# nanoshimarobot/dynamic_direct_lidar_odometry

Hardware: AMD Instinct MI355X
Metric: GICP iters/sec + ms/scan, 131k-pt source → 500k-pt submap; pose Δ vs CPU ref (higher is better)
Workload: dtype f32 search / f64 normal equations; 1 GPU; cfg3 S2M GICP: 131,072-pt 64x2048 scan -> 500,000-pt 4-keyframe submap, LM, maxCorr 2.0 m, maxIter 32, transEps 0.01; target_points=500000, parallelism=replicas x1

## Files before the change

dynamic_direct_lidar_odometry_amd/csrc/align.hip:

```cpp
#include <hip/hip_runtime.h>

#include <algorithm>
#include <array>
#include <atomic>
#include <cfloat>
#include <cmath>
#include <cstdlib>
#include <cstring>
#include <string>
#include <thread>
#include <vector>

#include "capi_internal.hpp"
#include "cellgrid.hpp"
#include "comm.hpp"

namespace {

constexpr float kSplitExtentDefault = 5.0f;
float env_float(const char* name, float dflt) {
  const char* v = dev_getenv(name);
  if (!v || !*v) return dflt;
  char* end = nullptr;
  const float f = std::strtof(v, &end);
  return (end && end != v && f >= 0.f) ? f : dflt;
}

int env_int(const char* name, int dflt) {
  const char* v = dev_getenv(name);
  return (v && *v) ? std::atoi(v) : dflt;
}

struct SearchKnobs {
  float split_extent, probe, probe_d, tri_mv, reuse_gap, reuse_gap0, reuse_rec_eps, reuse_rec_conv;
  int xcd_scan, pf_ratio, prev_window, reuse, reuse_rec0, tie_scan, tie_ab;
};
const SearchKnobs& search_knobs() {
  static const SearchKnobs k = [] {
    SearchKnobs v;
    v.split_extent = env_float("DDLO_SPLIT_EXTENT", kSplitExtentDefault);
    v.xcd_scan = env_int("DDLO_XCD_SCAN", 1);
    v.pf_ratio = env_int("DDLO_PF_RATIO", 2);
    v.prev_window = env_int("DDLO_PREV_WINDOW", 2);
    v.tri_mv = env_float("DDLO_TRI_MV", 0.2f);
    v.probe = env_float("DDLO_PROBE", 1.0f);
    v.probe_d = env_float("DDLO_PROBE_D", 0.5f);
    v.reuse = env_int("DDLO_REUSE", 1);
    v.reuse_gap = env_float("DDLO_REUSE_GAP", 0.05f);
    v.reuse_gap0 = env_float("DDLO_REUSE_GAP0", 0.f);
    v.reuse_rec0 = env_int("DDLO_REUSE_REC0", 0);
    v.reuse_rec_eps = env_float("DDLO_REUSE_REC_EPS", 0.05f);
    v.reuse_rec_conv = env_float("DDLO_REUSE_REC_CONV", 10.f);
    v.tie_ab = env_int("DDLO_TIE_AB", 0);
    v.tie_scan = env_int("DDLO_TIE_SCAN", 4);
    return v;
  }();
  return k;
}

constexpr int kMaxFirstChunk = 8;
constexpr int kMaxFixedChunk = 64;

}

float ddlo::rt::search_cap2(const gicp_params& p) {
  const double r = p.max_correspondence_distance;
  float f = (float)(r * r);
  if (!std::isfinite(f)) f = FLT_MAX;
  return std::nextafter(f, INFINITY);
}

bool ddlo::rt::grid_active(const gicp_ctx* c) {
  if (!c->grid_mode || !c->tgt.cloud) return false;
  const auto& g = c->tgt.cloud->grid;
  return g && g->ok && g->cap2 == search_cap2(c->params);
}

void ddlo::rt::finalize_job(gicp_ctx* c) {
  AlignJob& j = *c->job_host;
  j.job_full = 0;
  AlignJob probe = j;
  std::memcpy(probe.guess_R, c->job_last.guess_R, sizeof(probe.guess_R));
  std::memcpy(probe.guess_t, c->job_last.guess_t, sizeof(probe.guess_t));
  probe.job_full = c->job_last.job_full;
  probe.ticket = c->job_last.ticket;
  if (!c->job_last_valid || std::memcmp(&probe, &c->job_last, sizeof(AlignJob)) != 0) {
    j.job_full = 1;
    c->job_last = j;
    c->job_last_valid = true;
  }
}

gicp_status ddlo::rt::fill_job(gicp_ctx* c, const float* guess16, int nblocks) {
  const SearchKnobs& kn = search_knobs();
  AlignJob& j = *c->job_host;
  std::memset(&j, 0, sizeof(j));
  j.src = c->src.cloud->dev();
  j.tgt = c->tgt.cloud->dev();
  j.src_cov = c->src.cov->cov6.as<double>();
  j.tgt_cov = c->tgt.cov->cov6.as<double>();
  j.corr = c->corr.as<int>();
  j.sqd = c->sqd.as<float>();
  j.slab = c->slab.as<double>();
  j.state = c->state_dev.as<AlignState>();
  j.ticket = (++c->ticket) & ((1ull << 47) - 1);
  j.stats = c->stats_on ? c->stats.as<unsigned int>() : nullptr;
  for (int r = 0; r < 3; ++r) {
    for (int cc = 0; cc < 3; ++cc) j.guess_R[3 * r + cc] = guess16 ? (double)guess16[4 * r + cc] : (r == cc ? 1.0 : 0.0);
    j.guess_t[r] = guess16 ? (double)guess16[4 * r + 3] : 0.0;
  }
  const double r = c->params.max_correspondence_distance;
  j.max_corr2 = r * r;
  j.cap2 = search_cap2(c->params);
  j.nblocks = nblocks;
  j.fixed_iterations = c->params.fixed_iterations;
  j.max_iterations = c->params.fixed_iterations > 0 ? c->params.fixed_iterations : c->params.max_iterations;
  j.optimizer = c->params.optimizer;
  j.lm_max_iterations = c->params.lm_max_iterations;
  j.lm_init_lambda_factor = c->params.lm_init_lambda_factor;
  j.transformation_epsilon = c->params.transformation_epsilon;
  j.rotation_epsilon = c->params.rotation_epsilon;
  j.own_axis = c->own_axis;
  j.own_lo = c->own_lo;
  j.own_hi = c->own_hi;
  j.own_mod = c->own_mod;
  j.own_rem = c->own_rem;
  j.split_extent = kn.split_extent;
  j.premom = c->comm ? 1 : 0;
  j.mom = c->mom.as<double>();
  {
    const SearchLayout sl(c->src.cloud->n);
    char* u = c->search.as<char>();
    j.qstate = reinterpret_cast<float4*>(u + sl.qstate);
    j.key = reinterpret_cast<unsigned long long*>(u + sl.key);
    j.task_ctr = reinterpret_cast<unsigned*>(u + sl.ctr);
    j.tasks = reinterpret_cast<unsigned long long*>(u + sl.tasks);
    j.task_cap_r = sl.cap_r;
    j.ref = reinterpret_cast<float4*>(u + sl.ref);
    j.ref_p = reinterpret_cast<float4*>(u + sl.ref_p);
    j.sec = reinterpret_cast<unsigned*>(u + sl.sec);
    j.key2 = reinterpret_cast<unsigned long long*>(u + sl.key2);
  }
  j.xcd_scan = kn.xcd_scan;
  j.pf_ratio = kn.pf_ratio;
  j.prev_window = kn.prev_window;
  j.tri_mv = kn.tri_mv;
  j.probe2 = kn.probe * kn.probe;
  j.probe_d = kn.probe_d;
  j.reuse = kn.reuse;
  j.reuse_gap = kn.reuse_gap;
  j.reuse_gap0 = kn.reuse_gap0;
  j.cap2_d = (double)j.cap2;
  j.tri_mv_d = (double)j.tri_mv;
  j.reuse_gap_d = (double)j.reuse_gap;
  j.reuse_gap0_d = (double)j.reuse_gap0;
  j.reuse_rec0 = kn.reuse_rec0;
  j.reuse_rec_eps = kn.reuse_rec_eps;
  j.reuse_rec_conv = kn.reuse_rec_conv;
  j.tie_detect = (c->tie_exact && (c->own_axis < 0 || c->tie_tree)) ? 1 : 0;
  j.tgt_nf = NfTreeDev{nullptr, nullptr, nullptr, 0};
  j.tgt_nf_status = nullptr;
  j.tie_scan = j.tie_detect ? kn.tie_scan : 0;
  j.tie_ab = kn.tie_ab;
  if (j.tie_detect) {
    const NfTreeData* tt = c->tie_tree ? c->tie_tree.get() : c->tgt.cloud->nf.get();
    if (tt) {
      j.tgt_nf = tt->dev();
      j.tgt_nf_status = tt->status.as<int>();
    }
  }
  j.grid_on = grid_active(c) ? 1 : 0;
  if (j.grid_on) {
    j.task_cap_r = 0;
    j.grid = c->tgt.cloud->grid->dev;
    const FbLayout fl(c->src.cloud->n);
    char* u = c->fb.as<char>();
    j.fb_count = reinterpret_cast<unsigned*>(u + fl.ctr);
    j.fb_list = reinterpret_cast<int*>(u + fl.list);
    j.fb_seg_cap = fl.seg_cap;
    j.fb_mask = reinterpret_cast<unsigned short*>(u + fl.mask);
  }
  return GICP_OK;
}

namespace {

LinGeom geometry(const gicp_ctx* c) {
  LinGeom g = linearize_geometry(c->src.cloud->n, c->tgt.cloud->upper_count());
  g.state = c->state_dev.as<AlignState>();
  g.grid = grid_active(c);
  g.grid_walk = !g.grid || c->tgt.cloud->grid->dev.has_fallback != 0;
  g.fuse_lm = !c->comm && lm_fusion_enabled(g.grid && !g.grid_walk);
  return g;
}

}

gicp_status ddlo::rt::prepare_align(gicp_ctx* c) {
  if (!c->src.cloud) return fail(GICP_ENOSOURCE, "no source cloud");
  if (!c->tgt.cloud) return fail(GICP_ENOTARGET, "no target cloud");
  if (!c->src.has_cov()) {
    gicp_status s = compute_cov(c, c->src);
    if (s) return s;
  }
  if (!c->tgt.has_cov()) {
    gicp_status s = compute_cov(c, c->tgt);
    if (s) return s;
  }
  const int ns = c->src.cloud->n;
  const size_t need_corr = sizeof(int) * ns, need_sqd = sizeof(float) * ns,
               need_slab = sizeof(double) * kSlabStride * linearize_blocks(ns),
               need_search = SearchLayout(ns).total, need_fb = grid_active(c) ? FbLayout(ns).total : 0;
  if (need_corr > c->corr.bytes || need_sqd > c->sqd.bytes || need_slab > c->slab.bytes ||
      need_search > c->search.bytes || need_fb > c->fb.bytes ||
      (c->stats_on && sizeof(unsigned int) * kStatFields * (ns + 15) > c->stats.bytes)) {
    gicp_status s = drain_tail(c);
    if (s) return s;
  }
  HIP_TRY(c->corr.ensure(sizeof(int) * ns));
  HIP_TRY(c->sqd.ensure(sizeof(float) * ns));
  HIP_TRY(c->slab.ensure(sizeof(double) * kSlabStride * linearize_blocks(ns)));
  HIP_TRY(c->mom.ensure(sizeof(double) * kSlabStride));
  HIP_TRY(c->search.ensure(need_search));
  if (need_fb) HIP_TRY(c->fb.ensure(need_fb));
  if (c->tie_exact && (c->own_axis < 0 || c->tie_tree)) {
    CloudData& tc = *c->tgt.cloud;
    if (c->comm && !c->tie_tree && !tc.nf) {
      gicp_status s = ensure_nftree(c, tc, c->stream);
      if (s) return s;
    }
    const auto& nf = c->tie_tree ? c->tie_tree : tc.nf;
    if (nf && c->nf_joined.lock() != nf) {
      HIP_TRY(nftree_join(*nf, c->stream));
      c->nf_joined = nf;
    }
  }
  if (c->stats_on) {
    HIP_TRY(c->stats.ensure(sizeof(unsigned int) * kStatFields * (ns + 15)));
    HIP_TRY(hipMemsetAsync(c->stats.p, 0, c->stats.bytes, c->stream));
  }
  return GICP_OK;
}

gicp_status ddlo::rt::ensure_tie_tree(gicp_ctx* c) {
  gicp_status s = drain_tail(c);
  if (s) return s;
  s = ensure_nftree(c, *c->tgt.cloud, c->stream);
  if (s) return s;
  HIP_TRY(nftree_join(*c->tgt.cloud->nf, c->stream));
  c->nf_joined = c->tgt.cloud->nf;
  return GICP_OK;
}

gicp_status ddlo::rt::enqueue_iteration(gicp_ctx* c, const AlignJob* jd, int nblocks, AlignState* publish) {
  (void)nblocks;
  const LinGeom g = geometry(c);
  launch_linearize(c->stream, jd, g, publish);
  if (c->comm) {
    launch_mom_reduce(c->stream, jd);
    NCCL_TRY(rccl().all_reduce(c->mom.p, c->mom.p, kSlabStride, ncclFloat64, ncclSum, c->comm, c->stream));
  }
  if (!g.fuse_lm)
    launch_lm_step(c->stream, jd, c->state_dev.as<AlignState>(), c->slab.as<double>(), g.mom_blocks,
                   c->comm ? c->mom.as<double>() : nullptr, publish);
  return GICP_OK;
}

namespace {

gicp_status enqueue_chunk(gicp_ctx* c, bool with_init, int iters, int nblocks, int slot) {
  AlignJob* jd = c->job_dev.as<AlignJob>();
  if (with_init) launch_align_init(c->stream, jd, c->job_host_dev);
  for (int i = 0; i < iters; ++i) {
    gicp_status s = enqueue_iteration(c, jd, nblocks, i == iters - 1 ? c->state_host_dev + slot : nullptr);
    if (s) return s;
  }
  return GICP_OK;
}

gicp_status capture_chunk(gicp_ctx* c, bool with_init, int iters, int nblocks, int slot, hipExecGraphPair* out) {
  ++c->captures;
  HIP_TRY(hipStreamBeginCapture(c->stream, hipStreamCaptureModeThreadLocal));
  const gicp_status s = enqueue_chunk(c, with_init, iters, nblocks, slot);
  const hipError_t e = hipStreamEndCapture(c->stream, &out->g);
  if (s) return s;
  HIP_TRY(e);
  HIP_TRY(hipGraphInstantiate(&out->ge, out->g, nullptr, nullptr, 0));
  return GICP_OK;
}

void drop_pair(hipExecGraphPair& p) {
  if (p.ge) (void)hipGraphExecDestroy(p.ge);
  if (p.g) (void)hipGraphDestroy(p.g);
  p.ge = nullptr;
  p.g = nullptr;
}

void drop_set(GraphSet& gs) {
  for (auto& p : gs.first) drop_pair(p);
  gs.first.clear();
  drop_pair(gs.rest[0]);
  drop_pair(gs.rest[1]);
  gs.key.fill(-1);
}

}

void ddlo::rt::drop_graphs(gicp_ctx* c) {
  for (auto& gs : c->gsets) drop_set(gs);
  c->gsets.clear();
}

namespace {

gicp_status graph_set(gicp_ctx* c, const std::array<long long, 7>& key, int nblocks, GraphSet** out);

bool fresh_start_enabled() {
  static const bool on = [] {
    const char* v = dev_getenv("DDLO_FRESH_START");
    return !(v && *v == '0');
  }();
  return on;
}

bool fresh_start_allowed(const gicp_ctx* c, bool prev_ok, int max_it) {
  if (!prev_ok || !fresh_start_enabled() || c->job_host->job_full != 0 || max_it <= 0) return false;
  if (c->comm || c->profiling || c->stats_on) return false;
  const LinGeom g = geometry(c);
  return linearize_is_one_kernel(g) && g.fuse_lm;
}

gicp_status run_align_graph(gicp_ctx* c, int max_it, int nblocks, bool fresh, int* final_chunk) {
  const void* jd = c->job_dev.p;
  const LinGeom g = geometry(c);
  (void)nblocks;
  const std::array<long long, 7> key{{(long long)(uintptr_t)c->slab.p | (c->comm ? 1 : 0), (long long)(uintptr_t)jd,
                                      g.seed_blocks, g.scan_blocks, g.mom_blocks, g.lds_boxes,
                                      g.grid ? (g.grid_walk ? 2L : 1L) * g.lookup_blocks : 0}};
  const bool use_graph = !c->comm || c->comm_graphs;
  const int first = c->params.fixed_iterations > 0
                        ? std::max(1, std::min(max_it, kMaxFixedChunk))
                        : std::max(1, std::min({c->predicted_iters, max_it, kMaxFirstChunk}));
  GraphSet* gs = nullptr;
  if (use_graph) {
    gicp_status s = graph_set(c, key, nblocks, &gs);
    if (s) {
      drop_graphs(c);
      (void)hipGetLastError();
      if (!c->comm) return s;
      c->comm_graphs = false;
      return run_align_graph(c, max_it, nblocks, fresh, final_chunk);
    }
  }
  if (use_graph && !fresh && !gs->first[first - 1].ge) {
    gicp_status s = capture_chunk(c, true, first, nblocks, 0, &gs->first[first - 1]);
    if (s) {
      drop_graphs(c);
      return s;
    }
  }
  auto launch_chunk = [&](int k) -> gicp_status {
    const bool is_first = k == 0;
    if (is_first && fresh) {
      const AlignJob& jh = *c->job_host;
      FreshStart fs{};
      std::memcpy(fs.R, jh.guess_R, sizeof(fs.R));
      std::memcpy(fs.t, jh.guess_t, sizeof(fs.t));
      fs.ticket = jh.ticket;
      fs.job_w = c->job_dev.as<AlignJob>();
      fs.rec0 = jh.reuse && jh.reuse_rec0;
      launch_linearize_fresh(c->stream, c->job_dev.as<AlignJob>(), g, fs, first == 1 ? c->state_host_dev : nullptr);
      HIP_TRY(hipGetLastError());
      return first > 1 ? enqueue_chunk(c, false, first - 1, nblocks, 0) : GICP_OK;
    }
    if (use_graph) {
      HIP_TRY(hipGraphLaunch(is_first ? gs->first[first - 1].ge : gs->rest[k & 1].ge, c->stream));
      return GICP_OK;
    }
    return enqueue_chunk(c, is_first, is_first ? first : 1, nblocks, k & 1);
  };
  const int nchunks = 1 + (max_it - first);
  while ((int)c->chunk_ev.size() < nchunks) {
    hipEvent_t e;
    HIP_TRY(hipEventCreateWithFlags(&e, hipEventDisableTiming));
    c->chunk_ev.push_back(e);
  }
  gicp_status s = launch_chunk(0);
  if (s) return s;
  HIP_TRY(hipEventRecord(c->chunk_ev[0], c->stream));
  int launched = 1;
  if (nchunks > 1 && c->speculate) {
    s = launch_chunk(1);
    if (s) return s;
    HIP_TRY(hipEventRecord(c->chunk_ev[1], c->stream));
    launched = 2;
  }
  int k = 0;
  static const bool spin = [] {
    const char* v = dev_getenv("DDLO_SPIN_WAIT");
    return !(v && *v == '0');
  }();
  const unsigned long long ticket = c->job_host->ticket;
  for (;;) {
    if (spin) {
      static std::atomic<int> waiters{0};
      waiters.fetch_add(1, std::memory_order_relaxed);
      const volatile unsigned long long* pw = &(c->state_host + (k & 1))->pub;
      const int expect = first + k;
      hipError_t q = hipErrorNotReady;
      for (unsigned n = 1;; ++n) {
        const unsigned long long w = *pw;
        if ((w >> 17) == ticket && (((w >> 16) & 1ull) || (int)(w & 0xffffu) >= expect)) {
          q = hipSuccess;
          break;
        }
        if ((n & 63) == 0) {
          q = hipEventQuery(c->chunk_ev[k]);
          if (q != hipErrorNotReady) {
            const unsigned long long w2 = *pw;
            if (q == hipSuccess && !((w2 >> 17) == ticket && (((w2 >> 16) & 1ull) || (int)(w2 & 0xffffu) >= expect)))
              q = hipErrorUnknown;
            break;
          }
        }
        if (waiters.load(std::memory_order_relaxed) > 1) std::this_thread::yield();
      }
      waiters.fetch_sub(1, std::memory_order_relaxed);
      if (q == hipErrorUnknown) return fail(GICP_EHIP, "align chunk completed without its state publication");
      HIP_TRY(q);
    } else {
      HIP_TRY(hipEventSynchronize(c->chunk_ev[k]));
    }
    const volatile AlignState* st = c->state_host + (k & 1);
    if (st->done || k == nchunks - 1) break;
    while (launched < nchunks && launched <= k + 2) {
      s = launch_chunk(launched);
      if (s) return s;
      HIP_TRY(hipEventRecord(c->chunk_ev[launched], c->stream));
      ++launched;
    }
    ++k;
  }
  *final_chunk = k;
  c->state_slot = k & 1;
  c->tail_ev = c->chunk_ev[launched - 1];
  c->tail_pending = launched - 1 > k || spin;
  c->speculate = k > 0;
  c->predicted_iters = std::max(1, (int)((const volatile AlignState*)(c->state_host + (k & 1)))->iter);
  return GICP_OK;
}

gicp_status graph_set(gicp_ctx* c, const std::array<long long, 7>& key, int nblocks, GraphSet** out) {
  ++c->graph_clock;
  for (auto& gs : c->gsets)
    if (gs.key == key) {
      gs.last_use = c->graph_clock;
      *out = &gs;
      return GICP_OK;
    }
  GraphSet* slot = nullptr;
  if ((int)c->gsets.size() < kGraphSets) {
    c->gsets.reserve(kGraphSets);
    c->gsets.emplace_back();
    slot = &c->gsets.back();
  } else {
    slot = &c->gsets[0];
    for (auto& gs : c->gsets)
      if (gs.last_use < slot->last_use) slot = &gs;
    gicp_status s = drain_tail(c);
    if (s) return s;
    drop_set(*slot);
  }
  slot->first.resize(kMaxFixedChunk);
  gicp_status s = capture_chunk(c, false, 1, nblocks, 0, &slot->rest[0]);
  if (!s) s = capture_chunk(c, false, 1, nblocks, 1, &slot->rest[1]);
  if (s) return s;
  slot->key = key;
  slot->last_use = c->graph_clock;
  *out = slot;
  return GICP_OK;
}

gicp_status run_align_eager_profiled(gicp_ctx* c, int max_it, int nblocks) {
  AlignJob* jd = c->job_dev.as<AlignJob>();
  const size_t need = 2 * (size_t)max_it;
  while (c->prof_ev.size() < need) {
    hipEvent_t e;
    HIP_TRY(hipEventCreate(&e));
    c->prof_ev.push_back(e);
  }
  launch_align_init(c->stream, jd, c->job_host_dev);
  for (int i = 0; i < max_it; ++i) {
    HIP_TRY(hipEventRecord(c->prof_ev[2 * i], c->stream));
    LinGeom g = geometry(c);
    g.fuse_lm = false;
    launch_linearize(c->stream, jd, g);
    HIP_TRY(hipEventRecord(c->prof_ev[2 * i + 1], c->stream));
    if (c->comm) {
      launch_mom_reduce(c->stream, jd);
      NCCL_TRY(rccl().all_reduce(c->mom.p, c->mom.p, kSlabStride, ncclFloat64, ncclSum, c->comm, c->stream));
    }
    launch_lm_step(c->stream, jd, c->state_dev.as<AlignState>(), c->slab.as<double>(), g.mom_blocks,
                   c->comm ? c->mom.as<double>() : nullptr, nullptr);
  }
  HIP_TRY(hipGetLastError());
  return GICP_OK;
}

}

namespace ddlo {
bool lm_fusion_enabled(bool lookup) {
  static const int on = [] {
    const char* v = dev_getenv("DDLO_FUSE_LM");
    return v && *v ? std::atoi(v) : -1;
  }();
  return on < 0 ? lookup : on != 0;
}
}

extern "C" {

gicp_status gicp_align(gicp_ctx* c, const float* guess16, float* out16, gicp_result* res) {
  if (!c) return fail(GICP_EINVAL, "null ctx");
  bool prev_ok = c->fresh_ok;
  c->fresh_ok = false;
  c->dbg_search = false;
  bool graph_path = false;
  begin_ties(c);
  gicp_status s = set_device(c);
  if (s) return s;
  s = maybe_build_grid(c);
  if (s) return s;
  s = prepare_align(c);
  if (s) return s;
  const int ns = c->src.cloud->n;
  const int nblocks = linearize_blocks(ns);
  hipEvent_t end_ev = c->ev1;
  int reruns = 0;
  for (;;) {
    s = fill_job(c, guess16, nblocks);
    if (s) return s;
    finalize_job(c);
    JobCommit commit(c);
    const int max_it = c->job_host->max_iterations;
    const bool fresh = fresh_start_allowed(c, prev_ok, max_it);
    prev_ok = false;
    ++(fresh ? c->fresh_aligns : c->init_aligns);
    end_ev = c->ev1;
    if (c->profiling) HIP_TRY(hipEventRecord(c->ev0, c->stream));
    if (c->profiling || max_it <= 0) {
      s = max_it > 0 ? run_align_eager_profiled(c, max_it, nblocks) : GICP_OK;
      if (s) return s;
      if (max_it <= 0) launch_align_init(c->stream, c->job_dev.as<AlignJob>(), c->job_host_dev);
      HIP_TRY(hipGetLastError());
      commit.done();
      HIP_TRY(hipEventRecord(c->ev1, c->stream));
      HIP_TRY(hipMemcpyAsync(c->state_host, c->state_dev.p, sizeof(AlignState), hipMemcpyDeviceToHost, c->stream));
      HIP_TRY(hipStreamSynchronize(c->stream));
      c->state_slot = 0;
      c->tail_pending = false;
      graph_path = false;
    } else {
      int fc = 0;
      s = run_align_graph(c, max_it, nblocks, fresh, &fc);
      if (s) return s;
      commit.done();
      graph_path = true;
      end_ev = c->chunk_ev[fc];
    }
    if (!final_state(c).tie_pending || reruns > 0) break;
    s = ensure_tie_tree(c);
    if (s) return s;
    ++reruns;
  }
  const AlignState& st = final_state(c);
  c->have_align = st.iter > 0;
  c->last_nsrc = ns;
  if (out16) {
    for (int r = 0; r < 3; ++r) {
      for (int cc = 0; cc < 3; ++cc) out16[4 * r + cc] = (float)st.R[3 * r + cc];
      out16[4 * r + 3] = (float)st.t[r];
    }
    out16[12] = out16[13] = out16[14] = 0.f;
    out16[15] = 1.f;
  }
  if (res) {
    std::memset(res, 0, sizeof(*res));
    res->converged = st.converged;
    res->nr_iterations = st.nr_iterations;
    res->iterations_run = st.iter;
    res->lm_failed = st.lm_failed;
    res->lm_trials = st.lm_trials;
    res->num_correspondences = st.num_corr;
    res->final_cost = st.final_cost;
    std::memcpy(res->final_hessian, st.final_hessian, sizeof(res->final_hessian));
    res->lm_lambda = st.lambda;
    res->ties_resolved = st.ties_resolved;
    res->tie_reruns = reruns;
    if (c->profiling) {
      float ms = 0.f;
      HIP_TRY(hipEventSynchronize(end_ev));
      HIP_TRY(hipEventElapsedTime(&ms, c->ev0, end_ev));
      res->device_ms = ms;
      double tot = 0.0;
      for (int i = 0; i < st.iter; ++i) {
        float m = 0.f;
        HIP_TRY(hipEventElapsedTime(&m, c->prof_ev[2 * i], c->prof_ev[2 * i + 1]));
        tot += m;
      }
      res->linearize_ms = tot;
    }
  }
  s = check_ties(c);
  if (s) return s;
  if (st.tie_err || st.tie_pending)
    return fail(GICP_EHIP, "nanoflann tie order: a tied correspondence could not be re-run (bits " +
                               std::to_string(st.tie_err) + (st.tie_pending ? ", no tree" : "") + ")");
  if (st.lm_failed) g_last_error = "lm not converged!!";
  c->fresh_ok = graph_path && !st.tie_pending && !st.ties_resolved && !st.tie_err;
  return GICP_OK;
}

gicp_status gicp_linearize(gicp_ctx* c, const double* pose16, double* H36, double* b6, double* cost, int32_t* ncorr) {
  if (!c || !pose16) return fail(GICP_EINVAL, "null argument");
  c->fresh_ok = false;
  c->dbg_search = false;
  begin_ties(c);
  gicp_status s = set_device(c);
  if (s) return s;
  s = maybe_build_grid(c);
  if (s) return s;
  s = prepare_align(c);
  if (s) return s;
  const int ns = c->src.cloud->n;
  const int nblocks = linearize_blocks(ns);
  for (int rerun = 0;; ++rerun) {
    float g[16];
    for (int i = 0; i < 16; ++i) g[i] = 0.f;
    s = fill_job(c, g, nblocks);
    if (s) return s;
    for (int r = 0; r < 3; ++r) {
      for (int cc = 0; cc < 3; ++cc) c->job_host->guess_R[3 * r + cc] = pose16[4 * r + cc];
      c->job_host->guess_t[r] = pose16[4 * r + 3];
    }
    c->job_host->optimizer = GICP_OPT_GAUSS_NEWTON;
    c->job_host->max_iterations = 1;
    c->job_host->fixed_iterations = 1;
    finalize_job(c);
    JobCommit commit(c);
    AlignJob* jd = c->job_dev.as<AlignJob>();
    launch_align_init(c->stream, jd, c->job_host_dev);
    s = enqueue_iteration(c, jd, nblocks, nullptr);
    if (s) return s;
    HIP_TRY(hipGetLastError());
    commit.done();
    HIP_TRY(hipMemcpyAsync(c->state_host, c->state_dev.p, sizeof(AlignState), hipMemcpyDeviceToHost, c->stream));
    HIP_TRY(hipStreamSynchronize(c->stream));
    c->state_slot = 0;
    c->tail_pending = false;
    if (!final_state(c).tie_pending || rerun > 0) break;
    s = ensure_tie_tree(c);
    if (s) return s;
  }
  const AlignState& st = final_state(c);
  if (st.tie_err || st.tie_pending)
    return fail(GICP_EHIP, "nanoflann tie order: a tied correspondence could not be re-run (bits " +
                               std::to_string(st.tie_err) + ")");
  if (H36) std::memcpy(H36, st.final_hessian, sizeof(double) * 36);
  if (cost) *cost = st.final_cost;
  if (ncorr) *ncorr = st.num_corr;
  if (b6) std::memcpy(b6, st.last_b, sizeof(double) * 6);
  c->have_align = true;
  c->last_nsrc = ns;
  return GICP_OK;
}

}

gicp_status gicp_s2s_batch(int device, const gicp_params* p, const float* const* clouds, const size_t* sizes,
                           size_t stride_bytes, int nframes, int nstreams, float* out16, gicp_result* res) {
  if (!p || !clouds || !sizes || !out16 || nframes < 1 || nstreams < 1)
    return fail(GICP_EINVAL, "invalid batch arguments");
  for (int t = 0; t < nframes; ++t)
    if (!clouds[t] || sizes[t] == 0) return fail(GICP_EINVAL, "null or empty frame");
  for (int e = 0; e < 16; ++e) out16[e] = (e % 5 == 0) ? 1.f : 0.f;
  if (res) std::memset(&res[0], 0, sizeof(gicp_result));
  const int npairs = nframes - 1;
  if (npairs == 0) return GICP_OK;
  const int nthreads = std::min(nstreams, npairs);
  std::vector<gicp_status> status(nthreads, GICP_OK);
  std::vector<std::string> errors(nthreads);
  std::vector<gicp_ctx*> ctxs(nthreads, nullptr);
  for (int w = 0; w < nthreads; ++w) {
    gicp_status s = gicp_ctx_create(device, &ctxs[w]);
    if (!s) s = gicp_set_params(ctxs[w], p);
    if (!s) {
      const char* os = dev_getenv("DDLO_NF_OWN_STREAM");
      ctxs[w]->nf_same_stream = !(os && *os == '0');
    }
    if (s) {
      const std::string why = g_last_error;
      for (auto* c : ctxs)
        if (c) (void)gicp_ctx_destroy(c);
      return fail(s, why);
    }
  }
  auto worker = [&](int w) {
    const int t0 = 1 + (int)((long)npairs * w / nthreads);
    const int t1 = 1 + (int)((long)npairs * (w + 1) / nthreads);
    gicp_ctx* c = ctxs[w];
    gicp_status s = gicp_set_target(c, clouds[t0 - 1], sizes[t0 - 1], stride_bytes);
    for (int t = t0; t < t1 && !s; ++t) {
      s = set_source_impl(c, clouds[t], sizes[t], stride_bytes, 1, true);
      if (!s) s = gicp_align(c, nullptr, out16 + 16 * (size_t)t, res ? &res[t] : nullptr);
      if (!s) s = gicp_swap_source_target(c);
    }
    if (s) {
      status[w] = s;
      errors[w] = g_last_error;
    }
  };
  std::vector<std::thread> pool;
  for (int w = 1; w < nthreads; ++w) pool.emplace_back(worker, w);
  worker(0);
  for (auto& th : pool) th.join();
  for (auto* c : ctxs) (void)gicp_ctx_destroy(c);
  for (int w = 0; w < nthreads; ++w)
    if (status[w]) return fail(status[w], "s2s batch chunk " + std::to_string(w) + ": " + errors[w]);
  return GICP_OK;
}
```

dynamic_direct_lidar_odometry_amd/csrc/capi_debug.hip:

```cpp
#include <hip/hip_runtime.h>

#include <algorithm>
#include <cstddef>
#include <cstring>
#include <limits>
#include <string>
#include <vector>

#include "capi_internal.hpp"
#include "cellgrid.hpp"

extern "C" {

gicp_status gicp_debug_search_begin(gicp_ctx* c) {
  if (!c) return fail(GICP_EINVAL, "null ctx");
  c->fresh_ok = false;
  c->dbg_search = false;
  begin_ties(c);
  gicp_status s = set_device(c);
  if (s) return s;
  s = maybe_build_grid(c);
  if (s) return s;
  s = prepare_align(c);
  if (s) return s;
  const int ns = c->src.cloud->n;
  s = fill_job(c, nullptr, linearize_blocks(ns));
  if (s) return s;
  c->job_host->optimizer = GICP_OPT_GAUSS_NEWTON;
  c->job_host->max_iterations = 1 << 30;
  c->job_host->fixed_iterations = 1 << 30;
  c->job_last_valid = false;
  finalize_job(c);
  JobCommit commit(c);
  launch_align_init(c->stream, c->job_dev.as<AlignJob>(), c->job_host_dev);
  HIP_TRY(hipGetLastError());
  HIP_TRY(hipMemcpyAsync(c->state_host, c->state_dev.p, sizeof(AlignState), hipMemcpyDeviceToHost, c->stream));
  HIP_TRY(hipStreamSynchronize(c->stream));
  c->state_slot = 0;
  c->tail_pending = false;
  c->have_align = false;
  c->last_nsrc = ns;
  std::memcpy(&c->dbg_job, c->job_host, sizeof(AlignJob));
  c->dbg_search = true;
  return GICP_OK;
}

static gicp_status debug_search_job_current(gicp_ctx* c) {
  if (!c->src.cloud || !c->tgt.cloud || !c->src.has_cov() || !c->tgt.has_cov() || c->src.cloud->n != c->last_nsrc)
    return fail(GICP_ESTATE, "the clouds or covariances changed since gicp_debug_search_begin");
  const unsigned long long ticket = c->ticket;
  gicp_status s = fill_job(c, nullptr, linearize_blocks(c->src.cloud->n));
  c->ticket = ticket;
  if (s) return s;
  AlignJob& j = *c->job_host;
  j.optimizer = c->dbg_job.optimizer;
  j.max_iterations = c->dbg_job.max_iterations;
  j.fixed_iterations = c->dbg_job.fixed_iterations;
  j.job_full = c->dbg_job.job_full;
  j.ticket = c->dbg_job.ticket;
  const bool same = std::memcmp(&j, &c->dbg_job, sizeof(AlignJob)) == 0;
  std::memcpy(&j, &c->dbg_job, sizeof(AlignJob));
  if (!same) {
    c->dbg_search = false;
    return fail(GICP_ESTATE, "the ctx changed since gicp_debug_search_begin (parameters, covariances, shard, cells or tie tree): begin again");
  }
  return GICP_OK;
}

gicp_status gicp_debug_search_step(gicp_ctx* c, const double* pose16, int rec, double* H36, double* b6, double* cost,
                                   int32_t* ncorr) {
  if (!c || !pose16) return fail(GICP_EINVAL, "null argument");
  if (!c->dbg_search || !c->src.cloud || !c->tgt.cloud || c->src.cloud->n != c->last_nsrc)
    return fail(GICP_ESTATE, "gicp_debug_search_begin first");
  gicp_status s = set_device(c);
  if (s) return s;
  s = debug_search_job_current(c);
  if (s) return s;
  begin_ties(c);
  const int ns = c->src.cloud->n;
  const int nblocks = linearize_blocks(ns);
  AlignJob* jd = c->job_dev.as<AlignJob>();
  char* const sd = c->state_dev.as<char>();
  struct {
    double Rt[12];
    int done, rec;
  } w;
  for (int r = 0; r < 3; ++r) {
    for (int cc = 0; cc < 3; ++cc) w.Rt[3 * r + cc] = pose16[4 * r + cc];
    w.Rt[9 + r] = pose16[4 * r + 3];
  }
  w.done = 0;
  w.rec = rec ? 1 : 0;
  static_assert(offsetof(AlignState, t) == offsetof(AlignState, R) + 72, "R, t: 12 consecutive doubles");
  const bool may_rerun = c->job_host->tie_detect && !c->job_host->tgt_nf.nodes;
  const SearchLayout sl(ns);
  const size_t nb_state = align256(sizeof(AlignState)), nb_corr = align256(sizeof(int) * (size_t)ns),
               nb_search = sl.tasks;
  if (may_rerun) HIP_TRY(c->dbg_snap.ensure(nb_state + 2 * nb_corr + nb_search));
  char* const snap = c->dbg_snap.as<char>();
  auto carry = [&](bool save) -> gicp_status {
    const struct {
      void* p;
      size_t off, n;
    } part[4] = {{c->state_dev.p, 0, sizeof(AlignState)},
                 {c->corr.p, nb_state, sizeof(int) * (size_t)ns},
                 {c->sqd.p, nb_state + nb_corr, sizeof(float) * (size_t)ns},
                 {c->search.p, nb_state + 2 * nb_corr, nb_search}};
    for (const auto& q : part)
      HIP_TRY(hipMemcpyAsync(save ? (void*)(snap + q.off) : q.p, save ? q.p : (void*)(snap + q.off), q.n,
                             hipMemcpyDeviceToDevice, c->stream));
    return GICP_OK;
  };
  for (int rerun = 0;; ++rerun) {
    if (may_rerun) {
      s = carry(rerun == 0);
      if (s) return s;
    }
    HIP_TRY(hipMemcpyAsync(sd + offsetof(AlignState, R), w.Rt, sizeof(w.Rt), hipMemcpyHostToDevice, c->stream));
    HIP_TRY(hipMemcpyAsync(sd + offsetof(AlignState, done), &w.done, sizeof(int), hipMemcpyHostToDevice, c->stream));
    HIP_TRY(hipMemcpyAsync(sd + offsetof(AlignState, rec), &w.rec, sizeof(int), hipMemcpyHostToDevice, c->stream));
    s = enqueue_iteration(c, jd, nblocks, nullptr);
    if (s) return s;
    HIP_TRY(hipGetLastError());
    HIP_TRY(hipMemcpyAsync(c->state_host, c->state_dev.p, sizeof(AlignState), hipMemcpyDeviceToHost, c->stream));
    HIP_TRY(hipStreamSynchronize(c->stream));
    c->state_slot = 0;
    if (!final_state(c).tie_pending || rerun > 0 || !may_rerun) break;
    s = ensure_tie_tree(c);
    if (s) return s;
    const NfTreeData* tt = c->tgt.cloud->nf.get();
    c->job_host->tgt_nf = tt->dev();
    c->job_host->tgt_nf_status = tt->status.as<int>();
    HIP_TRY(hipMemcpyAsync(reinterpret_cast<char*>(jd) + offsetof(AlignJob, tgt_nf_status), &c->job_host->tgt_nf_status,
                           sizeof(c->job_host->tgt_nf_status), hipMemcpyHostToDevice, c->stream));
    HIP_TRY(hipMemcpyAsync(reinterpret_cast<char*>(jd) + offsetof(AlignJob, tgt_nf), &c->job_host->tgt_nf,
                           sizeof(NfTreeDev), hipMemcpyHostToDevice, c->stream));
    std::memcpy(&c->dbg_job, c->job_host, sizeof(AlignJob));
  }
  const AlignState& st = final_state(c);
  s = check_ties(c);
  if (s) return s;
  if (st.tie_err || st.tie_pending)
    return fail(GICP_EHIP, "nanoflann tie order: a tied correspondence could not be re-run (bits " +
                               std::to_string(st.tie_err) + ")");
  if (H36) std::memcpy(H36, st.final_hessian, sizeof(double) * 36);
  if (cost) *cost = st.final_cost;
  if (ncorr) *ncorr = st.num_corr;
  if (b6) std::memcpy(b6, st.last_b, sizeof(double) * 6);
  c->have_align = true;
  return GICP_OK;
}

gicp_status gicp_debug_search_state(gicp_ctx* c, int32_t* corr, float* sqd, uint32_t* sec, float* ref4, float* refp4,
                                    float* wr, int32_t* any_rec_out, size_t n) {
  if (!c) return fail(GICP_EINVAL, "null ctx");
  if (!c->have_align || !c->src.cloud || !c->tgt.cloud) return fail(GICP_ESTATE, "no linearization");
  if ((int)n != c->src.cloud->n || c->last_nsrc != (int)n) return fail(GICP_EINVAL, "n != source size");
  gicp_status s = set_device(c);
  if (s) return s;
  const SearchLayout sl(c->src.cloud->n);
  if (c->search.bytes < sl.total) return fail(GICP_ESTATE, "no search state");
  const int nt = c->tgt.cloud->n;
  std::vector<int> sperm(n), tperm((size_t)nt), hcorr(n);
  std::vector<float> hsqd(n);
  std::vector<unsigned> hsec(n);
  std::vector<float4> href(n), hrefp(n), hq(n);
  const char* u = c->search.as<char>();
  HIP_TRY(hipStreamSynchronize(c->stream));
  int any_rec = 0;
  HIP_TRY(hipMemcpy(&any_rec, c->state_dev.as<char>() + offsetof(AlignState, any_rec), sizeof(int), hipMemcpyDeviceToHost));
  if (any_rec_out) *any_rec_out = any_rec;
  HIP_TRY(hipMemcpy(sperm.data(), c->src.cloud->perm.p, sizeof(int) * n, hipMemcpyDeviceToHost));
  HIP_TRY(hipMemcpy(tperm.data(), c->tgt.cloud->perm.p, sizeof(int) * (size_t)nt, hipMemcpyDeviceToHost));
  HIP_TRY(hipMemcpy(hcorr.data(), c->corr.p, sizeof(int) * n, hipMemcpyDeviceToHost));
  HIP_TRY(hipMemcpy(hsqd.data(), c->sqd.p, sizeof(float) * n, hipMemcpyDeviceToHost));
  HIP_TRY(hipMemcpy(hsec.data(), u + sl.sec, sizeof(unsigned) * n, hipMemcpyDeviceToHost));
  HIP_TRY(hipMemcpy(href.data(), u + sl.ref, sizeof(float4) * n, hipMemcpyDeviceToHost));
  HIP_TRY(hipMemcpy(hrefp.data(), u + sl.ref_p, sizeof(float4) * n, hipMemcpyDeviceToHost));
  HIP_TRY(hipMemcpy(hq.data(), u + sl.qstate, sizeof(float4) * n, hipMemcpyDeviceToHost));
  for (size_t i = 0; i < n; ++i) {
    const size_t o = (size_t)sperm[i];
    if (o >= n) return fail(GICP_EHIP, "source permutation out of range");
    if (corr) corr[o] = (hcorr[i] >= 0 && hcorr[i] < nt) ? tperm[(size_t)hcorr[i]] : -1;
    if (sqd) sqd[o] = hsqd[i];
    if (sec) sec[o] = hsec[i];
    if (ref4) std::memcpy(ref4 + 4 * o, &href[i], sizeof(float4));
    if (refp4) {
      int j;
      std::memcpy(&j, &hrefp[i].w, sizeof(int));
      const int jo = (j >= 0 && j < nt) ? tperm[(size_t)j] : -1;
      refp4[4 * o] = hrefp[i].x;
      refp4[4 * o + 1] = hrefp[i].y;
      refp4[4 * o + 2] = hrefp[i].z;
      std::memcpy(refp4 + 4 * o + 3, &jo, sizeof(int));
    }
    if (wr) wr[o] = hq[i].w;
  }
  return GICP_OK;
}

gicp_status gicp_get_start_counts(gicp_ctx* c, int64_t* fresh_starts, int64_t* init_starts) {
  if (!c) return fail(GICP_EINVAL, "null ctx");
  if (fresh_starts) *fresh_starts = c->fresh_aligns;
  if (init_starts) *init_starts = c->init_aligns;
  return GICP_OK;
}

gicp_status gicp_get_lookup_stats(gicp_ctx* c, int64_t* walk_groups) {
  if (!c || !walk_groups) return fail(GICP_EINVAL, "null argument");
  *walk_groups = -1;
  if (!c->fb.p || !c->src.cloud) return GICP_OK;
  gicp_status s = set_device(c);
  if (s) return s;
  unsigned v = 0;
  const FbLayout fl(c->src.cloud->n);
  HIP_TRY(hipMemcpyAsync(&v, c->fb.as<char>() + fl.ctr + sizeof(unsigned) * kFbSegs * 32, sizeof(unsigned),
                         hipMemcpyDeviceToHost, c->stream));
  HIP_TRY(hipStreamSynchronize(c->stream));
  *walk_groups = v;
  return GICP_OK;
}

gicp_status gicp_debug_nftree(gicp_ctx* c, int side, int32_t* vind, int32_t* nodes4, float* div2, size_t cap,
                              size_t* nnodes) {
  if (!c || (side != 0 && side != 1) || !nnodes) return fail(GICP_EINVAL, "invalid argument");
  Side& sd = side == GICP_SIDE_SOURCE ? c->src : c->tgt;
  if (!sd.cloud) return fail(GICP_ESTATE, "no cloud on this side");
  gicp_status s = set_device(c);
  if (s) return s;
  s = ensure_nftree(c, *sd.cloud, c->stream);
  if (s) return s;
  const NfTreeData& t = *sd.cloud->nf;
  HIP_TRY(nftree_join(t, c->stream));
  int st[2] = {0, 0};
  HIP_TRY(hipMemcpyAsync(st, t.status.p, sizeof(st), hipMemcpyDeviceToHost, c->stream));
  HIP_TRY(hipStreamSynchronize(c->stream));
  if (st[0]) return fail(GICP_EHIP, "nanoflann tree build failed (error bits " + std::to_string(st[0]) + ")");
  *nnodes = (size_t)st[1];
  if (!vind && !nodes4 && !div2) return GICP_OK;
  if (cap < (size_t)st[1]) return fail(GICP_EINVAL, "node capacity too small");
  const int n = t.n;
  DevBuf dv, dn, df;
  HIP_TRY(dv.ensure(sizeof(int) * (size_t)n));
  HIP_TRY(dn.ensure(sizeof(int) * 4 * (size_t)st[1]));
  HIP_TRY(df.ensure(sizeof(float) * 2 * (size_t)st[1]));
  launch_nf_export(c->stream, t.dev(), t.status.as<int>(), st[1], dv.as<int>(), dn.as<int>(), df.as<float>());
  HIP_TRY(hipGetLastError());
  if (vind) HIP_TRY(hipMemcpyAsync(vind, dv.p, sizeof(int) * (size_t)n, hipMemcpyDeviceToHost, c->stream));
  if (nodes4) HIP_TRY(hipMemcpyAsync(nodes4, dn.p, sizeof(int) * 4 * (size_t)st[1], hipMemcpyDeviceToHost, c->stream));
  if (div2) HIP_TRY(hipMemcpyAsync(div2, df.p, sizeof(float) * 2 * (size_t)st[1], hipMemcpyDeviceToHost, c->stream));
  HIP_TRY(hipStreamSynchronize(c->stream));
  return GICP_OK;
}

gicp_status gicp_debug_nfbuild(gicp_ctx* c, int side, int stop, int32_t* vind, int64_t* info16, int32_t* status2,
                               void* scratch, size_t scratch_cap) {
  if (!c || (side != 0 && side != 1) || !vind || !info16 || !status2) return fail(GICP_EINVAL, "invalid argument");
  Side& sd = side == GICP_SIDE_SOURCE ? c->src : c->tgt;
  if (!sd.cloud) return fail(GICP_ESTATE, "no cloud on this side");
  gicp_status s = set_device(c);
  if (s) return s;
  NfTreeData t;
  long long off[16];
  s = nftree_build(c, *sd.cloud, c->stream, t, stop, off);
  if (s) return s;
  HIP_TRY(nftree_join(t, c->stream));
  for (int i = 0; i < 16; ++i) info16[i] = off[i];
  HIP_TRY(hipMemcpyAsync(status2, t.status.p, 2 * sizeof(int), hipMemcpyDeviceToHost, c->stream));
  std::vector<float4> v((size_t)t.n);
  HIP_TRY(hipMemcpyAsync(v.data(), t.vpts.p, sizeof(float4) * (size_t)t.n, hipMemcpyDeviceToHost, c->stream));
  if (scratch && scratch_cap)
    HIP_TRY(hipMemcpyAsync(scratch, c->nf_scratch.p, std::min(scratch_cap, (size_t)off[13]), hipMemcpyDeviceToHost,
                           c->stream));
  HIP_TRY(hipStreamSynchronize(c->stream));
  for (int i = 0; i < t.n; ++i) {
    int w;
    std::memcpy(&w, &v[(size_t)i].w, sizeof(int));
    vind[i] = w;
  }
  return GICP_OK;
}

gicp_status gicp_get_moments(const gicp_ctx* c, double* out80) {
  if (!c || !out80) return fail(GICP_EINVAL, "null argument");
  std::memcpy(out80, final_state(c).last_mom, sizeof(double) * kSlabStride);
  return GICP_OK;
}

gicp_status gicp_debug_lm_step(gicp_ctx* c, const gicp_lm_state* in, const double* slab, int nrows, const double* mom80,
                               gicp_lm_state* out) {
  if (!c || !in || !out || !slab == !mom80) return fail(GICP_EINVAL, "null argument (pass either slab or mom80)");
  const int max_rows = lm_slab_rows_max();
  if (slab && (nrows < 1 || nrows > max_rows)) return fail(GICP_EINVAL, "nrows must be in [1, 256]");
  gicp_status s = set_device(c);
  if (s) return s;
  AlignJob j{};
  j.fixed_iterations = c->params.fixed_iterations;
  j.max_iterations = c->params.fixed_iterations > 0 ? c->params.fixed_iterations : c->params.max_iterations;
  j.optimizer = c->params.optimizer;
  j.lm_max_iterations = c->params.lm_max_iterations;
  j.lm_init_lambda_factor = c->params.lm_init_lambda_factor;
  j.transformation_epsilon = c->params.transformation_epsilon;
  j.rotation_epsilon = c->params.rotation_epsilon;
  j.reuse = 0;
  AlignState st{};
  std::memcpy(st.R, in->R, sizeof(st.R));
  std::memcpy(st.t, in->t, sizeof(st.t));
  st.lambda = in->lambda;
  st.final_cost = in->final_cost;
  std::memcpy(st.final_hessian, in->final_hessian, sizeof(st.final_hessian));
  std::memcpy(st.last_b, in->last_b, sizeof(st.last_b));
  std::memcpy(st.last_mom, in->last_mom, sizeof(st.last_mom));
  st.iter = in->iter;
  st.lm_trials = in->lm_trials;
  st.converged = in->converged;
  st.lm_failed = in->lm_failed;
  st.done = 0;
  st.nr_iterations = in->nr_iterations;
  st.num_corr = in->num_corr;
  std::vector<double> rows;
  if (slab) {
    rows.assign((size_t)max_rows * kSlabStride, std::numeric_limits<double>::quiet_NaN());
    std::memcpy(rows.data(), slab, sizeof(double) * (size_t)nrows * kSlabStride);
  } else {
    rows.assign(mom80, mom80 + kSlabStride);
  }
  DevBuf djob, dstate, dmom;
  HIP_TRY(djob.ensure(sizeof(AlignJob)));
  HIP_TRY(dstate.ensure(sizeof(AlignState)));
  HIP_TRY(dmom.ensure(sizeof(double) * rows.size()));
  HIP_TRY(hipMemcpyAsync(djob.p, &j, sizeof(j), hipMemcpyHostToDevice, c->stream));
  HIP_TRY(hipMemcpyAsync(dstate.p, &st, sizeof(st), hipMemcpyHostToDevice, c->stream));
  HIP_TRY(hipMemcpyAsync(dmom.p, rows.data(), sizeof(double) * rows.size(), hipMemcpyHostToDevice, c->stream));
  launch_lm_step(c->stream, djob.as<AlignJob>(), dstate.as<AlignState>(), slab ? dmom.as<double>() : nullptr,
                 slab ? nrows : 0, slab ? nullptr : dmom.as<double>(), nullptr);
  HIP_TRY(hipGetLastError());
  HIP_TRY(hipMemcpyAsync(&st, dstate.p, sizeof(st), hipMemcpyDeviceToHost, c->stream));
  HIP_TRY(hipStreamSynchronize(c->stream));
  std::memcpy(out->R, st.R, sizeof(st.R));
  std::memcpy(out->t, st.t, sizeof(st.t));
  out->lambda = st.lambda;
  out->final_cost = st.final_cost;
  std::memcpy(out->final_hessian, st.final_hessian, sizeof(st.final_hessian));
  std::memcpy(out->last_b, st.last_b, sizeof(st.last_b));
  std::memcpy(out->last_mom, st.last_mom, sizeof(st.last_mom));
  out->iter = st.iter;
  out->lm_trials = st.lm_trials;
  out->converged = st.converged;
  out->lm_failed = st.lm_failed;
  out->done = st.done;
  out->nr_iterations = st.nr_iterations;
  out->num_corr = st.num_corr;
  out->reserved = 0;
  return GICP_OK;
}

gicp_status gicp_debug_stats(gicp_ctx* c, int enable, unsigned int* out, size_t max_words, size_t* nwords) {
  if (!c) return fail(GICP_EINVAL, "null ctx");
  c->stats_on = enable != 0;
  if (out && c->src.cloud && c->stats.p) {
    const int q = search_queries_per_wave();
    const size_t groups = (c->src.cloud->n + q - 1) / q;
    const size_t words = std::min(max_words, (size_t)kStatFields * (groups + (groups + 3) / 4));
    HIP_TRY(hipMemcpyAsync(out, c->stats.p, sizeof(unsigned int) * words, hipMemcpyDeviceToHost, c->stream));
    HIP_TRY(hipStreamSynchronize(c->stream));
    if (nwords) *nwords = words;
  }
  return GICP_OK;
}

gicp_status gicp_set_profiling(gicp_ctx* c, int enable) {
  if (!c) return fail(GICP_EINVAL, "null ctx");
  c->profiling = enable != 0;
  return GICP_OK;
}

gicp_status gicp_get_stage_times(gicp_ctx* c, gicp_stage_times* out) {
  if (!c || !out) return fail(GICP_EINVAL, "null argument");
  std::memset(out, 0, sizeof(*out));
  if (!c->st_ev[0]) return fail(GICP_ESTATE, "no profiled compute_covariances on this ctx");
  gicp_status s = set_device(c);
  if (s) return s;
  HIP_TRY(hipStreamSynchronize(c->stream));
  HIP_TRY(hipStreamSynchronize(c->aux_stream));
  float ms = 0.f;
  HIP_TRY(hipEventElapsedTime(&ms, c->st_ev[0], c->st_ev[1]));
  out->cov_ms = ms;
  if (c->st_tree) {
    HIP_TRY(hipEventElapsedTime(&ms, c->st_ev[2], c->st_ev[3]));
    out->tree_ms = ms;
  }
  if (c->st_resolve) {
    HIP_TRY(hipEventElapsedTime(&ms, c->st_ev[4], c->st_ev[5]));
    out->resolve_ms = ms;
  }
  return GICP_OK;
}

}
```

dynamic_direct_lidar_odometry_amd/csrc/capi_internal.hpp:

```cpp
#pragma once
#include "runtime.hpp"

namespace ddlo {
namespace rt {

struct SearchLayout {
  size_t qstate, key, ctr, ref, ref_p, sec, key2, tasks, total;
  int cap_r;
  explicit SearchLayout(int ns) {
    cap_r = task_cap_per_region(ns);
    qstate = 0;
    key = align256(sizeof(float4) * (size_t)ns);
    ctr = key + align256(sizeof(unsigned long long) * (size_t)ns);
    ref = ctr + align256(sizeof(unsigned) * (kTaskRegions + 1) * kCtrStride);
    ref_p = ref + align256(sizeof(float4) * (size_t)ns);
    sec = ref_p + align256(sizeof(float4) * (size_t)ns);
    key2 = sec + align256(sizeof(unsigned) * (size_t)ns);
    tasks = key2 + align256(sizeof(unsigned long long) * (size_t)ns);
    total = tasks + sizeof(unsigned long long) * (size_t)kTaskRegions * cap_r;
  }
};

struct FbLayout {
  size_t ctr, list, mask, total;
  int seg_cap;
  explicit FbLayout(int ns) {
    seg_cap = (ns + 15) / 16 + 1;
    ctr = 0;
    list = align256(sizeof(unsigned) * (kFbSegs + 1) * 32);
    mask = list + align256(sizeof(int) * (size_t)kFbSegs * seg_cap);
    total = mask + align256(sizeof(unsigned short) * (size_t)seg_cap);
  }
};


float search_cap2(const gicp_params& p);
bool grid_active(const gicp_ctx* c);

inline int linearize_blocks(int nsrc) { return linearize_geometry(nsrc, 0).mom_blocks; }

struct JobCommit {
  gicp_ctx* c;
  bool ok = false;
  explicit JobCommit(gicp_ctx* ctx) : c(ctx) {}
  void done() { ok = true; }
  ~JobCommit() {
    if (!ok) c->job_last_valid = c->fresh_ok = false;
  }
};
void finalize_job(gicp_ctx* c);
gicp_status fill_job(gicp_ctx* c, const float* guess16, int nblocks);
gicp_status prepare_align(gicp_ctx* c);
gicp_status ensure_tie_tree(gicp_ctx* c);
gicp_status enqueue_iteration(gicp_ctx* c, const AlignJob* jd, int nblocks, AlignState* publish);
void drop_graphs(gicp_ctx* c);


gicp_status set_source_impl(gicp_ctx* c, const float* xyz, size_t n, size_t stride, int build_index, bool nf_early);

}
}
```

dynamic_direct_lidar_odometry_amd/csrc/gicp_types.hpp:

```cpp
#pragma once
#include <stdint.h>

namespace ddlo {

constexpr int kLeafSize = 32;
constexpr int kFanout = 64;
constexpr int kMaxLevels = 5;
constexpr int kDirBits = 18;
constexpr int kFineBits = 6;
constexpr int kFineMin = 32;
__host__ __device__ constexpr long fine_dir_ints(int n) {
  return (1L << kDirBits) + 2 + (1L << kDirBits) + ((long)(n / (kFineMin + 1) + 1) << kFineBits) / 2;
}

constexpr int kMoments = 74;
constexpr int kMomentSlots = 96;
constexpr int kSlabStride = 80;
constexpr int kStatFields = 8;

constexpr int kTaskRegions = 64;
constexpr int kCtrStride = 32;
constexpr int kTasksPerGroup = 48;

struct CloudDev {
  const float4* pts;
  const unsigned long long* keys;
  const int* perm;
  const int* inv_perm;
  const float4* box_lo;
  const float4* box_hi;
  const float* quant;
  const float* soa;
  const int* dir;
  int n;
  int nlevels;
  int off0, off1, off2, off3, off4;
  int cnt0, cnt1, cnt2, cnt3, cnt4;
};

__host__ __device__ inline int lvl_off(const CloudDev& c, int l) {
  return l == 0 ? c.off0 : l == 1 ? c.off1 : l == 2 ? c.off2 : l == 3 ? c.off3 : c.off4;
}
__host__ __device__ inline int lvl_cnt(const CloudDev& c, int l) {
  return l == 0 ? c.cnt0 : l == 1 ? c.cnt1 : l == 2 ? c.cnt2 : l == 3 ? c.cnt3 : c.cnt4;
}

struct NfNode {
  int c1, c2;
  int feat;
  float divlow, divhigh;
  int parent;
  int pad0, pad1;
};

struct NfTreeDev {
  const float4* vpts;
  const NfNode* nodes;
  const float4* box;
  int n;
  int partial;
  const float4* sbox;
};

constexpr unsigned long long kCgNoMatch = ~0ull;
constexpr unsigned long long kCgFallback = ~0ull - 1;
constexpr unsigned kCgFineFallback = 0xffffffffu;
constexpr int kCgMaxLevel = 3;
constexpr int kCgEntPad = 32;

struct CellGridDev {
  const unsigned long long* dir;
  const uint2* fine;
  const float4* ent;
  float ox, oy, oz, inv_s;
  int nx, ny, nz;
  int outside_nomatch;
  int has_fallback;
};

__device__ __forceinline__ int cg_cell_list(const CellGridDev& G, float tx, float ty, float tz, unsigned& off,
                                            unsigned& cnt) {
  const int cx = min((int)tx, G.nx - 1), cy = min((int)ty, G.ny - 1), cz = min((int)tz, G.nz - 1);
  const unsigned long long d = G.dir[((long)cx * G.ny + cy) * G.nz + cz];
  if (d == kCgNoMatch) return 0;
  if (d == kCgFallback) return 2;
  const int lvl = (int)(d >> 62);
  unsigned long long e = d;
  if (lvl != 0) {
    const int m = 1 << lvl;
    const int fx = min((int)((tx - (float)cx) * (float)m), m - 1);
    const int fy = min((int)((ty - (float)cy) * (float)m), m - 1);
    const int fz = min((int)((tz - (float)cz) * (float)m), m - 1);
    e = reinterpret_cast<const unsigned long long*>(G.fine)[(unsigned)d + (unsigned)((fx * m + fy) * m + fz)];
  }
  if ((unsigned)(e >> 32) == kCgFineFallback) return 2;
  off = (unsigned)e;
  cnt = (unsigned)(e >> 32) & 0x3fffffffu;
  return 1;
}

struct AlignState {
  double R[9];
  double t[3];
  double lambda;
  double final_hessian[36];
  double final_cost;
  double last_lin_R[9];
  double last_lin_t[3];
  double last_b[6];
  double last_mom[kSlabStride];
  int iter;
  int done;
  int converged;
  int nr_iterations;
  int lm_failed;
  int lm_trials;
  int num_corr;
  int have_prev;
  int rec;
  float src_radius;
  int any_rec;
  int tie_pending;
  int ties_resolved;
  int tie_err;
  unsigned long long pub;
};

struct AlignJob {
  CloudDev src;
  CloudDev tgt;
  const double* src_cov;
  const double* tgt_cov;
  int* corr;
  float* sqd;
  double* slab;
  AlignState* state;
  unsigned int* stats;
  double guess_R[9];
  double guess_t[3];
  long long job_full;
  unsigned long long ticket;
  double max_corr2;
  float cap2;
  double cap2_d, tri_mv_d, reuse_gap_d, reuse_gap0_d;
  int nblocks;
  int max_iterations;
  int fixed_iterations;
  int optimizer;
  int lm_max_iterations;
  double lm_init_lambda_factor;
  double transformation_epsilon;
  double rotation_epsilon;
  int own_axis;
  float own_lo, own_hi;
  int own_mod, own_rem;
  int premom;
  double* mom;
  float split_extent;
  float4* qstate;
  unsigned long long* key;
  unsigned long long* tasks;
  unsigned* task_ctr;
  int task_cap_r;
  int xcd_scan;
  int pf_ratio;
  int prev_window;
  float probe2;
  float probe_d;
  float tri_mv;
  int reuse;
  float reuse_gap;
  float reuse_gap0;
  int reuse_rec0;
  float reuse_rec_eps;
  float reuse_rec_conv;
  float4* ref;
  float4* ref_p;
  unsigned* sec;
  unsigned long long* key2;
  int tie_detect;
  int tie_ab;
  int tie_scan;
  const int* tgt_nf_status;
  NfTreeDev tgt_nf;
  int grid_on;
  CellGridDev grid;
  unsigned* fb_count;
  int* fb_list;
  int fb_seg_cap;
  unsigned short* fb_mask;
};
constexpr int kFbSegs = 8;

struct FreshStart {
  double R[9];
  double t[3];
  unsigned long long ticket;
  AlignJob* job_w;
  int rec0;
};

constexpr int kNfMaxLevels = 40;
constexpr int kNfLevelSpare = 2;

struct NfCtl {
  int nnodes, nsmall, err;
  int nchunks[2];
  int ntask[kNfMaxLevels + 1];
  int dbg[16];
};

struct NfTask {
  int node, begin, count, chunk0;
  float lo[3], hi[3];
  unsigned mm[6];
  int feat;
  float cut;
  int nch, pad;
};

struct NfBuild {
  float4* vpts;
  NfNode* nodes;
  float4* box;
  int cap;
  NfCtl* ctl;
  NfTask* tasks;
  NfTask* pend;
  NfTask* small;
  int* chunk_task;
  NfTask* ctask;
  int *cA, *cAE, *cE2;
  float4 *tblL, *tblR;
  const float* quant;
  float4* sbox;
  const float4* sorted;
  const int* gate;
  int n, Lmax, max_task, max_pend, max_small, max_chunks;
  int nbucket;
  int big_ids;
};

struct NfSizes {
  int Lmax, max_task, max_pend, max_small, max_chunks, big_ids;
};

struct KnnJob {
  CloudDev c;
  int k;
  int method;
  double* cov6;
  float4* qstate;
  unsigned long long* cand;
  unsigned* cnt;
  int cap;
  unsigned long long* tasks;
  unsigned* task_ctr;
  int task_cap_r;
  unsigned char* redo;
  unsigned char* again;
  int round;
  int* slot2;
  unsigned long long* cand2;
  unsigned* n2;
  int cap2, max2;
  float split_extent;
  int* tie_list;
  int* tie_count;
  int tie_cap;
};

}
```

dynamic_direct_lidar_odometry_amd/csrc/launch.hpp:

```cpp
#pragma once
#include <hip/hip_runtime.h>

#include "gicp_types.hpp"

namespace ddlo {

void launch_pack_bbox(hipStream_t s, const unsigned char* raw, size_t stride, int n, float4* out, float* partial,
                      int* nonfinite, int nblocks);
void launch_bbox_final(hipStream_t s, const float* partial, int nparts, float* quant);
void launch_morton(hipStream_t s, const float4* pts, int n, const float* quant, unsigned long long* keys, int* vals);
void launch_gather(hipStream_t s, const float4* raw, const int* perm, int n, int npad, float4* sorted, int* inv_perm);
void launch_key_dir(hipStream_t s, const unsigned long long* keys, int n, int* dir);
void launch_leaf_soa_boxes(hipStream_t s, const float4* pts, int n, int nleaves, float* soa, float4* lo, float4* hi);
void launch_level_boxes(hipStream_t s, const float4* clo, const float4* chi, int nchild, int nparent, float4* plo,
                        float4* phi);
struct TieList {
  int* list;
  int* count;
  int cap = 0;
  __device__ __forceinline__ void push(int i) const {
    const int slot = atomicAdd(count, 1);
    if (slot < cap) list[slot] = i;
  }
};
bool launch_covariances(hipStream_t s, const CloudDev& c, int k, int method, double* cov6, const unsigned char* redo,
                        TieList ties = TieList{nullptr, nullptr});
bool launch_knn_covariances(hipStream_t s, const KnnJob& j, int tgt_upper);
int knn_task_cap_per_region(int n);
bool launch_knn_query(hipStream_t s, const CloudDev& c, const float4* q, int nq, int k, int* out_idx, float* out_d,
                      TieList ties = TieList{nullptr, nullptr});
void launch_cov_import(hipStream_t s, const double* in, int layout, int n, const int* inv_perm, double* cov6);
void launch_cov_export(hipStream_t s, const double* cov6, int layout, int n, const int* perm, double* out);
size_t tie_prune_scratch_bytes(int n, int cap);
hipError_t launch_tie_prune(hipStream_t s, const NfTreeDev& t, int cap, const int* local_index, int n_local,
                            void* scratch, NfNode* out_nodes, float4* out_pts, unsigned* counts);
void launch_align_init(hipStream_t s, AlignJob* job, const AlignJob* job_src);
struct LinGeom {
  int seed_blocks, scan_blocks, mom_blocks, lds_boxes, lookup_blocks;
  bool fuse_lm = false;
  AlignState* state = nullptr;
  bool grid = false;
  bool grid_walk = true;
};
bool lm_fusion_enabled(bool lookup);
LinGeom linearize_geometry(int nsrc, int tgt_upper);
void launch_linearize(hipStream_t s, const AlignJob* job, const LinGeom& g, AlignState* publish = nullptr);
bool linearize_is_one_kernel(const LinGeom& g);
void launch_linearize_fresh(hipStream_t s, const AlignJob* job, const LinGeom& g, const FreshStart& fs,
                            AlignState* publish = nullptr);
int search_queries_per_wave();
int task_cap_per_region(int nsrc);
int moment_blocks(int nsrc);
int lm_slab_rows_max();
void launch_lm_step(hipStream_t s, const AlignJob* job, AlignState* st, const double* slab, int nblocks,
                    const double* premom, AlignState* publish);
void launch_mom_reduce(hipStream_t s, const AlignJob* job);
void launch_residuals(hipStream_t s, const AlignJob* job, int nsrc, double* out);
void launch_residual_image(hipStream_t s, const float4* pts, const int* perm, const int* inv_perm, int n,
                           const double* residual, double tmin, double tmax, int W, int H, int* winner, float* img,
                           float* xyz);
void launch_transform(hipStream_t s, const float4* pts, int n, const int* perm, const float* T16, float* out,
                      size_t stride_floats);
void launch_export_corr(hipStream_t s, const AlignJob* job, int nsrc, int* corr, float* sqd);

NfSizes nf_sizes(int n);
void launch_nf_build(hipStream_t s, const NfBuild& hb, const NfBuild* db, int stop = -1);
void launch_nf_set_desc(hipStream_t s, const NfBuild& b, NfBuild* db);
void launch_nf_export(hipStream_t s, const NfTreeDev& t, const int* status, int cap, int* vind, int* nodes, float* f);
bool launch_nf_resolve_cov(hipStream_t s, const NfTreeDev& t, const CloudDev& c, TieList ties, int k, int method,
                           double* cov6, const int* status, int* err);
bool launch_nf_resolve_knn(hipStream_t s, const NfTreeDev& t, const float4* q, TieList ties, int k, int* out_idx,
                           float* out_d, const int* status, int* err);
size_t nf_lazy_bytes(int n, int wgs);
bool launch_nf_lazy(hipStream_t s, const NfTreeDev& t, const CloudDev& c, const float4* q, TieList ties, int k,
                    int method, double* cov6, int* out_idx, float* out_d, void* scratch, int wgs, const int* status,
                    int* err);
void launch_cov_remap(hipStream_t s, const double* old_cov6, const int* old_inv_perm, const int* new_perm, int n,
                      double* cov6);

void launch_pack4(hipStream_t s, const unsigned char* raw, size_t stride, int n, float4* out);
long long rowcol_size(int rows, int cols, int row_step, int col_step);
int rowcol_count(int n, int rows, int cols, int row_step, int col_step);
int launch_pack4_rowcol(hipStream_t s, const unsigned char* raw, size_t stride, int n, int rows, int cols, int row_step,
                        int col_step, float4* out);
struct CropCentre {
  float x = 0.f, y = 0.f, z = 0.f;
};
int crop_box(hipStream_t s, const float4* in, int n, float size, float4* out, int* keep, int* pos, void* tmp,
             size_t tmp_bytes, int* count_host, int* pin, CropCentre centre = CropCentre(), bool box = true);
size_t crop_box_tmp_bytes(int n);
int compact_flagged(hipStream_t s, const float4* in, int n, float4* out, const int* keep, int* pos, void* tmp,
                    size_t tmp_bytes, int* count_host, int* pin);
int voxel_grid(hipStream_t s, const float4* in, int n, float leaf, float4* out, int* scratch, void* tmp, size_t tmp_bytes,
               int* count_host, float crop, int* pin, CropCentre centre = CropCentre(), int order = 0,
               int* oscratch = nullptr);
size_t voxel_tmp_bytes(int n);
constexpr size_t voxel_scratch_ints(int n) { return 7 * (size_t)n + 16 + 6 * 64; }

constexpr int kVoxelOrderHandOver = 512;
size_t sort_order_scratch_ints(int n);
size_t voxel_order_scratch_ints(int n);
void launch_sort_order(hipStream_t s, unsigned* keys, int* idx, int n, const int* pos, const int* keep, int* scratch);
int voxel_order_pairs(hipStream_t s, const unsigned* keys, const int* idx, int n, int* oscratch, void* tmp,
                      size_t tmp_bytes, unsigned** ck_out, int** ci_out);
void median_range_async(hipStream_t s, const float4* in, int n, float* d, float* result, void* tmp, size_t tmp_bytes,
                        float* out);
size_t median_tmp_bytes(int n);
void launch_transform4(hipStream_t s, const float4* pts, const int* perm, int n, const float* T12, float4* out);
void launch_transform_raw(hipStream_t s, const unsigned char* raw, size_t stride, int n, const float* T12, float4* out);
void launch_gather_cov6(hipStream_t s, const double* cov_sorted, const int* perm, int n, double* out);

}
```

dynamic_direct_lidar_odometry_amd/csrc/lm_step.hpp:

```cpp
#pragma once
#include <hip/hip_runtime.h>

#include "gicp_types.hpp"
#include "search.hpp"

namespace ddlo {

static __device__ void so3_exp_d(const double w[3], double R[9]) {
  const double theta_sq = w[0] * w[0] + w[1] * w[1] + w[2] * w[2];
  double imag, real;
  if (theta_sq < 1e-10) {
    const double theta_quad = theta_sq * theta_sq;
    imag = 0.5 - 1.0 / 48.0 * theta_sq + 1.0 / 3840.0 * theta_quad;
    real = 1.0 - 1.0 / 8.0 * theta_sq + 1.0 / 384.0 * theta_quad;
  } else {
    const double theta = sqrt(theta_sq);
    const double half = 0.5 * theta;
    double sh, ch;
    sincos(half, &sh, &ch);
    imag = sh / theta;
    real = ch;
  }
  const double qw = real, qx = imag * w[0], qy = imag * w[1], qz = imag * w[2];
  const double tx = 2 * qx, ty = 2 * qy, tz = 2 * qz;
  const double twx = tx * qw, twy = ty * qw, twz = tz * qw;
  const double txx = tx * qx, txy = ty * qx, txz = tz * qx;
  const double tyy = ty * qy, tyz = tz * qy, tzz = tz * qz;
  R[0] = 1 - (tyy + tzz); R[1] = txy - twz;       R[2] = txz + twy;
  R[3] = txy + twz;       R[4] = 1 - (txx + tzz); R[5] = tyz - twx;
  R[6] = txz - twy;       R[7] = tyz + twx;       R[8] = 1 - (txx + tyy);
}

static __device__ void ldlt_solve6_perm(const double* H, const double* b, double lambda, double* xs, double x[6]) {
  constexpr int n = 6;
  double v[6];
  int p[6];
#pragma unroll
  for (int i = 0; i < n; ++i) {
    v[i] = fabs(H[7 * i] + lambda);
    p[i] = i;
  }
#pragma unroll
  for (int k = 0; k < n - 1; ++k) {
    double bv = v[k];
    int bp = p[k], big = k;
#pragma unroll
    for (int i = k + 1; i < n; ++i)
      if (v[i] > bv) { bv = v[i]; bp = p[i]; big = i; }
#pragma unroll
    for (int i = k + 1; i < n; ++i)
      if (big == i) { v[i] = v[k]; p[i] = p[k]; }
    v[k] = bv;
    p[k] = bp;
  }
  double m[36];
#pragma unroll
  for (int i = 0; i < n; ++i)
#pragma unroll
    for (int j = 0; j <= i; ++j) {
      const int hi = max(p[i], p[j]), lo = min(p[i], p[j]);
      m[i * n + j] = i == j ? H[7 * p[i]] + lambda : H[hi * n + lo];
    }
#pragma unroll
  for (int k = 0; k < n; ++k) {
    if (k > 0) {
      double temp[6];
#pragma unroll
      for (int j = 0; j < k; ++j) temp[j] = m[j * n + j] * m[k * n + j];
      double s = 0;
#pragma unroll
      for (int j = 0; j < k; ++j) s += m[k * n + j] * temp[j];
      m[k * n + k] -= s;
#pragma unroll
      for (int i = k + 1; i < n; ++i) {
        double a = 0;
#pragma unroll
        for (int j = 0; j < k; ++j) a += m[i * n + j] * temp[j];
        m[i * n + k] -= a;
      }
    }
    const double akk = m[k * n + k];
    if (k < n - 1 && fabs(akk) > 0.0) {
#pragma unroll
      for (int i = k + 1; i < n; ++i) m[i * n + k] /= akk;
    }
  }
  double y[6];
#pragma unroll
  for (int i = 0; i < n; ++i) y[i] = -b[p[i]];
#pragma unroll
  for (int i = 0; i < n; ++i)
#pragma unroll
    for (int j = 0; j < i; ++j) y[i] -= m[i * n + j] * y[j];
#pragma unroll
  for (int i = 0; i < n; ++i) y[i] = (fabs(m[i * n + i]) > 2.2250738585072014e-308) ? y[i] / m[i * n + i] : 0.0;
#pragma unroll
  for (int i = n - 1; i >= 0; --i)
#pragma unroll
    for (int j = i + 1; j < n; ++j) y[i] -= m[j * n + i] * y[j];
#pragma unroll
  for (int i = 0; i < n; ++i) xs[p[i]] = y[i];
#pragma unroll
  for (int i = 0; i < n; ++i) x[i] = xs[i];
}

constexpr int mom_ab(int a, int b) {
  return a <= b ? (a == 0 ? b : (a == 1 ? 2 + b : 5)) : (b == 0 ? a : (b == 1 ? 2 + a : 5));
}
constexpr int mom_w(int k, int l, int a, int b) {
  return (k == 3 && l == 3) ? mom_ab(a, b)
         : k == 3           ? 6 + 6 * l + mom_ab(a, b)
         : l == 3           ? 6 + 6 * k + mom_ab(a, b)
                            : 24 + 6 * mom_ab(k, l) + mom_ab(a, b);
}
constexpr int mom_g(int mm, int k) { return 60 + 4 * mm + k; }
constexpr int kMomY0 = 72, kMomCount = 73;

constexpr int kNeqEntries = 198;
struct NeqTerm {
  unsigned idx;
  unsigned sgn;
  unsigned ctl;
};
struct NeqTable {
  NeqTerm e[kNeqEntries];
};
constexpr void skew_nz_c(int i, int p, int& c, int& r, int& sg) {
  constexpr int cc[3][2] = {{1, 2}, {0, 2}, {0, 1}};
  constexpr int rr[3][2] = {{2, 1}, {2, 0}, {1, 0}};
  constexpr int ss[3][2] = {{-1, 1}, {1, -1}, {-1, 1}};
  c = cc[i][p];
  r = rr[i][p];
  sg = ss[i][p];
}
constexpr NeqTable make_neq_table() {
  NeqTable T{};
  auto add = [&](int e, int idx, int sg) {
    const unsigned t = T.e[e].ctl & 0xffu;
    T.e[e].idx |= (unsigned)idx << (8 * t);
    T.e[e].sgn |= (sg < 0 ? 0xffu : 1u) << (8 * t);
    T.e[e].ctl += 1u;
  };
  for (int e = 0; e < 42; ++e) {
    if (e >= 36) {
      const int i = e - 36;
      if (i >= 3) {
        add(e, mom_g(i - 3, 3), -1);
      } else {
        for (int p = 0; p < 2; ++p) {
          int c = 0, r = 0, sg = 0;
          skew_nz_c(i, p, c, r, sg);
          add(e, mom_g(r, c), sg);
        }
      }
      continue;
    }
    const int i = e / 6, j = e % 6;
    if (i < 3 && j < 3) {
      for (int p = 0; p < 2; ++p) {
        int c = 0, r = 0, sr = 0;
        skew_nz_c(i, p, c, r, sr);
        for (int u = 0; u < 2; ++u) {
          int d = 0, q = 0, sq = 0;
          skew_nz_c(j, u, d, q, sq);
          add(e, mom_w(c, d, r, q), sr * sq);
        }
      }
    } else if (i >= 3 && j >= 3) {
      add(e, mom_w(3, 3, i - 3, j - 3), 1);
    } else {
      const int a = i < 3 ? i : j, t = i < 3 ? j - 3 : i - 3;
      for (int p = 0; p < 2; ++p) {
        int c = 0, r = 0, sr = 0;
        skew_nz_c(a, p, c, r, sr);
        add(e, mom_w(c, 3, r, t), sr);
      }
      T.e[e].ctl |= 0x100u;
    }
  }
  for (int e = 0; e < 144; ++e) add(42 + e, mom_w(e / 12 / 3, e % 12 / 3, e / 12 % 3, e % 12 % 3), 1);
  for (int e = 0; e < 12; ++e) add(186 + e, mom_g(e % 3, e / 3), 1);
  return T;
}
static __constant__ NeqTable kNeq = make_neq_table();
__device__ __forceinline__ double neq_term(const NeqTerm& E, const double* mom, int t) {
  const double v = mom[(E.idx >> (8 * t)) & 0xffu];
  return ((E.sgn >> (8 * t)) & 0xffu) == 1u ? v : -v;
}
__device__ __forceinline__ double neq_value(const NeqTerm& E, const double* mom) {
  const unsigned n = E.ctl & 0xffu;
  double s = neq_term(E, mom, 0);
  if (n > 1) {
    s = 0.0 + s;
#pragma unroll
    for (int t = 1; t < 4; ++t)
      if (t < (int)n) s += neq_term(E, mom, t);
  }
  return (E.ctl & 0x100u) ? -s : s;
}

constexpr int kLmThreads = 512;
constexpr int kMaxTrials = 64;
constexpr int kMomBlocksMax = 256;
constexpr int kLmParts = 12;
constexpr int kLmRowsPerPart = (kMomBlocksMax + kLmParts - 1) / kLmParts;

__device__ __forceinline__ void reduce_slab(const double* slab_in, int nb, double (*part)[kSlabStride], double* mom) {
  const int tid = threadIdx.x;
  const auto slab = (const __attribute__((address_space(1))) d2v*)gp(slab_in);
  constexpr int kPairs = kSlabStride / 2;
  if (tid < kLmParts * kPairs) {
    const int v2 = tid % kPairs, p = tid / kPairs;
    d2v x[kLmRowsPerPart];
#pragma unroll
    for (int r = 0; r < kLmRowsPerPart; ++r) x[r] = slab[(size_t)min(p + kLmParts * r, nb - 1) * kPairs + v2];
    double s0 = 0.0, s1 = 0.0;
#pragma unroll
    for (int r = 0; r < kLmRowsPerPart; ++r) {
      const bool in = p + kLmParts * r < nb;
      s0 += in ? x[r].x : 0.0;
      s1 += in ? x[r].y : 0.0;
    }
    part[p][2 * v2] = s0;
    part[p][2 * v2 + 1] = s1;
  }
  __syncthreads();
  if (tid < kSlabStride) {
    double s = 0.0;
#pragma unroll
    for (int p = 0; p < kLmParts; ++p) s += part[p][tid];
    mom[tid] = s;
  }
}

#ifdef DDLO_LM_PROF
#define LM_PROF(i) if (threadIdx.x == 0) lm_t[i] = __builtin_amdgcn_s_memtime()
#define LM_PROF_TRIAL(i) if (threadIdx.x == 0) lm_tt[i] = __builtin_amdgcn_s_memtime()
#else
#define LM_PROF(i)
#define LM_PROF_TRIAL(i)
#endif
template <bool PREMOM, bool FRESH = false>
__device__ __forceinline__ void lm_step_body(const AlignJob* __restrict__ job, AlignState* __restrict__ st,
                                             const double* __restrict__ slab, int nblocks,
                                             const double* __restrict__ premom, const FreshStart* fs = nullptr) {
#ifdef DDLO_LM_PROF
  unsigned long long lm_t[6], lm_tt[4] = {0, 0, 0, 0};
#endif
  LM_PROF(0);
  __shared__ double part[kLmParts][kSlabStride];
  __shared__ double mom[kSlabStride];
  __shared__ double nq[kNeqEntries];
  double* const Hs = nq;
  double* const bs = nq + 36;
  double* const W12 = nq + 42;
  double* const g12 = nq + 186;
  __shared__ double tr_lambda[kMaxTrials], tr_cm[kMaxTrials], tr_fro[kMaxTrials];
  __shared__ double tr_R[kMaxTrials][9], tr_t[kMaxTrials][3];
  __shared__ double tr_d[kMaxTrials][12], tr_row[kMaxTrials][12], tr_den[kMaxTrials], tr_x[kMaxTrials][6];
  __shared__ double Rt_s[12];
  __shared__ int tr_conv[kMaxTrials];
  const int tid = threadIdx.x;
  const int it_pre = FRESH ? 0 : st->iter;
  const int trials_pre = FRESH ? 0 : st->lm_trials;
  const int rec_pre = FRESH ? fs->rec0 : st->rec;
  const float src_radius = st->src_radius;
  const double lambda_pre = FRESH ? -1.0 : st->lambda;
  double rt_v = 0.0;
  if constexpr (FRESH) {
#pragma unroll
    for (int e = 0; e < 12; ++e)
      if (tid == e) rt_v = e < 9 ? fs->R[e] : fs->t[e - 9];
  } else {
    if (tid < 12) rt_v = tid < 9 ? st->R[tid] : st->t[tid - 9];
  }
  const int optimizer = job->optimizer, lm_max_iterations = job->lm_max_iterations;
  const int fixed_iterations = job->fixed_iterations, max_iterations = job->max_iterations;
  const double lm_init_lambda_factor = job->lm_init_lambda_factor;
  const double rotation_epsilon = job->rotation_epsilon, transformation_epsilon = job->transformation_epsilon;
  const int reuse = job->reuse;
  const float reuse_rec_eps = job->reuse_rec_eps, reuse_rec_conv = job->reuse_rec_conv;
  NeqTerm E{};
  if (tid < kNeqEntries) E = kNeq.e[tid];
  if constexpr (PREMOM) {
    if (tid < kSlabStride) mom[tid] = gp(premom)[tid];
  } else {
    reduce_slab(slab, nblocks, part, mom);
  }
  if (tid < 12) Rt_s[tid] = rt_v;
  __syncthreads();
  LM_PROF(1);
  if (tid < kNeqEntries) nq[tid] = neq_value(E, mom);
  __syncthreads();
  LM_PROF(2);
  const bool lm = optimizer != 0;
  const int ntr = lm ? min(lm_max_iterations, kMaxTrials) : 1;
  if (tid < ntr) {
    const int trial = tid;
    double lambda = 0.0;
    if (lm) {
      lambda = lambda_pre;
      if (lambda < 0.0) {
        double mx = 0.0;
        for (int e = 0; e < 6; ++e) mx = fmax(mx, fabs(Hs[7 * e]));
        lambda = lm_init_lambda_factor * mx;
      }
      double nu = 2.0;
      for (int k = 0; k < trial; ++k) {
        lambda = nu * lambda;
        nu = 2 * nu;
      }
    }
    LM_PROF_TRIAL(0);
    double d[6];
    ldlt_solve6_perm(Hs, bs, lambda, tr_x[trial], d);
    LM_PROF_TRIAL(1);
    double Rd[9], td[3];
    so3_exp_d(d, Rd);
    LM_PROF_TRIAL(2);
    td[0] = d[3]; td[1] = d[4]; td[2] = d[5];
    double den = 0.0;
    for (int e = 0; e < 6; ++e) den += d[e] * (lambda * d[e] - bs[e]);
    tr_den[trial] = den;
    tr_lambda[trial] = lambda;
    double mr = 0.0, mt = 0.0;
    for (int i = 0; i < 3; ++i)
      for (int j = 0; j < 3; ++j) mr = fmax(mr, fabs(Rd[3 * i + j] - (i == j ? 1.0 : 0.0)));
    for (int i = 0; i < 3; ++i) mt = fmax(mt, fabs(td[i]));
    const double cm = fmax(1.0 / rotation_epsilon * mr, 1.0 / transformation_epsilon * mt);
    tr_cm[trial] = cm;
    tr_conv[trial] = fixed_iterations <= 0 && cm < 1;
    double fro = 0.0;
    for (int e = 0; e < 9; ++e) {
      const double dd = Rd[e] - ((e % 4 == 0) ? 1.0 : 0.0);
      fro += dd * dd;
    }
    tr_fro[trial] = fro;
    for (int e = 0; e < 9; ++e) tr_R[trial][e] = Rd[e];
    for (int e = 0; e < 3; ++e) tr_t[trial][e] = td[e];
#pragma unroll
    for (int k = 0; k < 4; ++k)
#pragma unroll
      for (int a = 0; a < 3; ++a) tr_d[trial][3 * k + a] = k < 3 ? Rd[3 * a + k] - (a == k ? 1.0 : 0.0) : td[a];
    LM_PROF_TRIAL(3);
  }
  __syncthreads();
  LM_PROF(3);
  for (int x = tid; lm && x < 12 * ntr; x += (int)blockDim.x) {
    const int tr = x / 12, i = x % 12;
    double srow = 0.0;
#pragma unroll
    for (int j = 0; j < 12; ++j) srow += W12[12 * i + j] * tr_d[tr][j];
    tr_row[tr][i] = tr_d[tr][i] * srow;
  }
  __syncthreads();
  LM_PROF(4);
  if (tid >= 64) {
    const int u = tid - 64;
    if (u < kSlabStride) st->last_mom[u] = mom[u];
    else if (u < kSlabStride + 9) st->last_lin_R[u - kSlabStride] = Rt_s[u - kSlabStride];
    else if (u < kSlabStride + 12) st->last_lin_t[u - kSlabStride - 9] = Rt_s[u - kSlabStride];
    else if (u < kSlabStride + 18) st->last_b[u - kSlabStride - 12] = bs[u - kSlabStride - 12];
    return;
  }
  const int lane = tid;
  double rho = 1.0;
  if (lm && lane < ntr) {
    double lin = 0.0, quad = 0.0;
#pragma unroll
    for (int r = 0; r < 3; ++r)
#pragma unroll
      for (int k = 0; k < 4; ++k) lin += tr_d[lane][3 * k + r] * g12[3 * k + r];
#pragma unroll
    for (int i = 0; i < 12; ++i) quad += tr_row[lane][i];
    rho = (2.0 * lin - quad) / tr_den[lane];
  }
  bool ok = true, accept = true;
  int chosen = 0;
  if (lm) {
    const unsigned long long ball = __ballot(lane < ntr && (!(rho < 0) || tr_conv[lane]));
    ok = ball != 0ull;
    chosen = ok ? (int)__builtin_ctzll(ball) : ntr - 1;
    const double rho_c = __shfl(rho, chosen);
    accept = ok && !(rho_c < 0);
    if (lane == 0) {
      st->lm_trials = trials_pre + (ok ? chosen + 1 : ntr);
      if (accept) {
        const double c = 2 * rho_c - 1;
        st->lambda = tr_lambda[chosen] * fmax(1.0 / 3.0, 1 - c * c * c);
      } else if (ok) {
        st->lambda = tr_lambda[chosen];
      } else {
        st->lambda = tr_lambda[ntr - 1] * 2.0;
      }
    }
  } else if (FRESH && lane == 0) {
    st->lm_trials = 0;
    st->lambda = -1.0;
  }
  if (lane == 0) {
    st->nr_iterations = it_pre;
    st->final_cost = mom[kMomY0];
    st->num_corr = (int)mom[kMomCount];
    if (rec_pre) st->any_rec = 1;
    else if (FRESH) st->any_rec = 0;
    st->iter = it_pre + 1;
    st->have_prev = 1;
    int done = 0;
    if constexpr (FRESH) {
      const int failed = !ok, conv = ok && tr_conv[chosen];
      st->lm_failed = failed;
      st->converged = conv;
      done = failed | conv;
      if (it_pre + 1 >= max_iterations) done = 1;
      st->done = done;
    } else {
      if (!ok) {
        st->lm_failed = 1;
        done = 1;
      } else if (tr_conv[chosen]) {
        st->converged = 1;
        done = 1;
      }
      if (it_pre + 1 >= max_iterations) done = 1;
      if (done) st->done = 1;
    }
  }
  double v = 0.0;
  if (accept) {
    const double* Rd = tr_R[chosen];
    if (lane < 9) {
      const int i = lane / 3, j = lane % 3;
      v = Rd[3 * i + 0] * Rt_s[0 + j] + Rd[3 * i + 1] * Rt_s[3 + j] + Rd[3 * i + 2] * Rt_s[6 + j];
      st->R[lane] = v;
    } else if (lane < 12) {
      const int i = lane - 9;
      v = (Rd[3 * i + 0] * Rt_s[9] + Rd[3 * i + 1] * Rt_s[10] + Rd[3 * i + 2] * Rt_s[11]) + tr_t[chosen][i];
      st->t[i] = v;
    } else if (lane >= 16 && lane < 16 + 36) {
      st->final_hessian[lane - 16] = Hs[lane - 16];
    }
  } else if (FRESH && lane < 12) {
    if (lane < 9) st->R[lane] = Rt_s[lane];
    else st->t[lane - 9] = Rt_s[lane];
  }
  int rec = reuse;
  if (accept) {
    const double tn0 = __shfl(v, 9), tn1 = __shfl(v, 10), tn2 = __shfl(v, 11);
    const double* dt = tr_t[chosen];
    const double mv = sqrt(tr_fro[chosen]) * ((double)src_radius + sqrt(tn0 * tn0 + tn1 * tn1 + tn2 * tn2)) +
                      sqrt(dt[0] * dt[0] + dt[1] * dt[1] + dt[2] * dt[2]);
    rec = rec && mv < (double)reuse_rec_eps && (fixed_iterations > 0 || tr_cm[chosen] > (double)reuse_rec_conv);
  }
  if (lane == 0) st->rec = rec;
  LM_PROF(5);
#ifdef DDLO_LM_PROF
  if (tid == 0)
    printf("lm_prof %d %llu %llu %llu %llu %llu %llu %llu %llu %llu\n", it_pre, lm_t[1] - lm_t[0], lm_t[2] - lm_t[1],
           lm_t[3] - lm_t[2], lm_t[4] - lm_t[3], lm_t[5] - lm_t[4], lm_tt[0] - lm_t[2], lm_tt[1] - lm_tt[0],
           lm_tt[2] - lm_tt[1], lm_tt[3] - lm_tt[2]);
#endif
}

}
```

dynamic_direct_lidar_odometry_amd/csrc/moments.hip:

```cpp
#include <hip/hip_runtime.h>

#include <cstddef>

#include "gicp_types.hpp"
#include "search.hpp"
#include "nftree.hpp"
#include "cov_math.hpp"
#include "launch.hpp"
#include "launch_util.hpp"
#include "linearize_internal.hpp"
#include "lm_step.hpp"

namespace ddlo {

struct Contrib {
  double M[6];
  double q[3];
  double qq[6];
  double v[3];
  double y;
  double c;
};

template <int S>
__device__ __forceinline__ double moment_val(const Contrib& C) {
  if constexpr (S < 6) {
    return C.M[S];
  } else if constexpr (S < 24) {
    return C.q[(S - 6) / 6] * C.M[(S - 6) % 6];
  } else if constexpr (S < 60) {
    return C.qq[(S - 24) / 6] * C.M[(S - 24) % 6];
  } else if constexpr (S < 72) {
    constexpr int m = (S - 60) / 4, kk = (S - 60) % 4;
    if constexpr (kk == 3)
      return C.v[m];
    else
      return C.v[m] * C.q[kk];
  } else if constexpr (S == 72) {
    return C.y;
  } else if constexpr (S == 73) {
    return C.c;
  } else {
    return 0.0;
  }
}

__device__ __forceinline__ double dpp_f64(double x, int ctrl_sel) {
  const int lo = __double2loint(x), hi = __double2hiint(x);
  int rlo, rhi;
  switch (ctrl_sel) {
    case 0:
      rlo = __builtin_amdgcn_update_dpp(0, lo, 0x140, 0xf, 0xf, false);
      rhi = __builtin_amdgcn_update_dpp(0, hi, 0x140, 0xf, 0xf, false);
      break;
    case 1:
      rlo = __builtin_amdgcn_update_dpp(0, lo, 0x141, 0xf, 0xf, false);
      rhi = __builtin_amdgcn_update_dpp(0, hi, 0x141, 0xf, 0xf, false);
      break;
    case 2:
      rlo = __builtin_amdgcn_update_dpp(0, lo, 0x4e, 0xf, 0xf, false);
      rhi = __builtin_amdgcn_update_dpp(0, hi, 0x4e, 0xf, 0xf, false);
      break;
    default:
      rlo = __builtin_amdgcn_update_dpp(0, lo, 0xb1, 0xf, 0xf, false);
      rhi = __builtin_amdgcn_update_dpp(0, hi, 0xb1, 0xf, 0xf, false);
      break;
  }
  return __hiloint2double(rhi, rlo);
}

template <int L>
__device__ __forceinline__ double xchg(double a, double b) {
  if constexpr (L == 1 || L == 2) {
    const unsigned alo = __double2loint(a), ahi = __double2hiint(a);
    const unsigned blo = __double2loint(b), bhi = __double2hiint(b);
    unsigned x0, x1, y0, y1;
    if constexpr (L == 1) {
      const auto rl = __builtin_amdgcn_permlane32_swap(alo, blo, false, false);
      const auto rh = __builtin_amdgcn_permlane32_swap(ahi, bhi, false, false);
      x0 = rl[0]; y0 = rl[1]; x1 = rh[0]; y1 = rh[1];
    } else {
      const auto rl = __builtin_amdgcn_permlane16_swap(alo, blo, false, false);
      const auto rh = __builtin_amdgcn_permlane16_swap(ahi, bhi, false, false);
      x0 = rl[0]; y0 = rl[1]; x1 = rh[0]; y1 = rh[1];
    }
    return __hiloint2double(x1, x0) + __hiloint2double(y1, y0);
  } else {
    const int bit = 1 << (6 - L);
    const bool hi = (lane_id() & bit) != 0;
    const double keep = hi ? b : a;
    const double send = hi ? a : b;
    return keep + dpp_f64(send, L - 3);
  }
}

template <int L, int S>
__device__ __forceinline__ double treduce(const Contrib& C) {
  if constexpr (L == 0) {
    return moment_val<S>(C);
  } else {
    constexpr int half = kMomentSlots >> L;
    const double a = treduce<L - 1, S>(C);
    const double b = treduce<L - 1, S + half>(C);
    return xchg<L>(a, b);
  }
}

__device__ __forceinline__ double final_pair(double x) { return x + dpp_f64(x, 3); }

__device__ __forceinline__ int moment_base(int lane) {
  return 48 * ((lane >> 5) & 1) + 24 * ((lane >> 4) & 1) + 12 * ((lane >> 3) & 1) + 6 * ((lane >> 2) & 1) +
         3 * ((lane >> 1) & 1);
}

__device__ __forceinline__ void load_sym6(const __attribute__((address_space(1))) double* p, double c[6]) {
  const auto q = (const __attribute__((address_space(1))) d2v*)p;
  const d2v a = q[0];
  const d2v b = q[1];
  const d2v d = q[2];
  c[0] = a.x; c[1] = a.y; c[2] = b.x; c[3] = b.y; c[4] = d.x; c[5] = d.y;
}

constexpr int kMomWaves = 8;

__device__ __forceinline__ void resolve_tied_corr(const AlignJob* __restrict__ job, AlignState* st, const CloudDev& tgt,
                                               bool tied, int i, float kd, int& j, NfWaveStack* S,
                                               bool q_in_regs = false, float qx = 0.f, float qy = 0.f, float qz = 0.f) {
  unsigned long long tm = __ballot(tied);
  const int lane = lane_id();
  const NfTreeDev t = job->tgt_nf;
  if (t.nodes == nullptr) {
    if (lane == __builtin_ctzll(tm)) atomicOr(&st->tie_pending, 1);
    return;
  }
  if (*job->tgt_nf_status) {
    if (lane == __builtin_ctzll(tm)) atomicOr(&st->tie_err, 2);
    return;
  }
  int nres = 0;
  while (tm) {
    const int l = __builtin_ctzll(tm);
    tm &= tm - 1;
    const int il = __builtin_amdgcn_readlane(i, l);
    const float dl = __uint_as_float((unsigned)__builtin_amdgcn_readlane((int)__float_as_uint(kd), l));
    const float4 q = q_in_regs ? make_float4(readlane_f(qx, l), readlane_f(qy, l), readlane_f(qz, l), 0.f)
                               : ldg4(job->qstate, il);
    float rd;
    int rix;
    int err = 0, jn = -1;
    const bool ok = nf_search_wave(t, q.x, q.y, q.z, 1, S, &rd, &rix);
    rd = __uint_as_float((unsigned)__builtin_amdgcn_readfirstlane((int)__float_as_uint(rd)));
    rix = __builtin_amdgcn_readfirstlane(rix);
    if (!ok) err = 1;
    else if (__float_as_uint(rd) != __float_as_uint(dl) || rix < 0 || rix >= t.n) err = 16;
    else if ((jn = tgt.inv_perm[rix]) < 0) err = 32;
    if (lane == l) {
      if (jn >= 0) j = jn;
      else atomicOr(&st->tie_err, err);
    }
    ++nres;
  }
  if (lane == 0) atomicAdd(&st->ties_resolved, nres);
}

#ifndef DDLO_LOOKUP_U
#define DDLO_LOOKUP_U 16
#endif
constexpr int kLookupU = DDLO_LOOKUP_U;
#ifndef DDLO_TAIL_E0
#define DDLO_TAIL_E0 32
#endif
#ifndef DDLO_TAIL_FCAP
#define DDLO_TAIL_FCAP 64
#endif
constexpr unsigned kTailE0 = DDLO_TAIL_E0;
constexpr int kTailFCap = DDLO_TAIL_FCAP;
static_assert(kTailE0 > 0 && kTailE0 % kLookupU == 0, "the common rounds end on a round boundary");
static_assert(kTailFCap >= 1 && kTailFCap <= 64 && (kTailFCap & (kTailFCap - 1)) == 0, "team size: a power of two");

constexpr unsigned kLookupInf = 0x7f800000u;
struct LookupBest {
  unsigned long long bk;
  unsigned d2;
};
__device__ __forceinline__ void tail_merge(LookupBest& a, const LookupBest& o) {
  const bool take = o.bk < a.bk;
  const unsigned long long loser = take ? a.bk : o.bk;
  if (take) a.bk = o.bk;
  a.d2 = min(min(a.d2, o.d2), (unsigned)(loser >> 32));
}
__device__ __forceinline__ LookupBest tail_shfl(const LookupBest& s, int src) {
  LookupBest r;
  r.bk = ((unsigned long long)(unsigned)__shfl((int)(unsigned)(s.bk >> 32), src) << 32) |
         (unsigned)__shfl((int)(unsigned)s.bk, src);
  r.d2 = (unsigned)__shfl((int)s.d2, src);
  return r;
}

#ifdef DDLO_MOM_PROF
#define MOM_PROF(i) if (LOOKUP) mp_t[i] = __builtin_amdgcn_s_memrealtime()
constexpr int kMomProfIters = 8, kMomProfWaves = 2048;
constexpr int kMomProfWords = 7;
__device__ unsigned long long g_mom_prof[kMomProfIters * kMomProfWaves * kMomProfWords];
#else
#define MOM_PROF(i)
#endif
struct TieWords {
  int pending, resolved, err;
};
constexpr int kTieThread = 64 * (kMomWaves - 1);
__device__ __forceinline__ TieWords fetch_tie_words(AlignState* st) {
  TieWords tw{0, 0, 0};
  __hip_atomic_compare_exchange_strong(&st->tie_pending, &tw.pending, 0, __ATOMIC_RELAXED, __ATOMIC_RELAXED,
                                       __HIP_MEMORY_SCOPE_AGENT);
  __hip_atomic_compare_exchange_strong(&st->ties_resolved, &tw.resolved, 0, __ATOMIC_RELAXED, __ATOMIC_RELAXED,
                                       __HIP_MEMORY_SCOPE_AGENT);
  __hip_atomic_compare_exchange_strong(&st->tie_err, &tw.err, 0, __ATOMIC_RELAXED, __ATOMIC_RELAXED,
                                       __HIP_MEMORY_SCOPE_AGENT);
  return tw;
}

__device__ __forceinline__ void publish_state(const AlignJob* __restrict__ job, AlignState* __restrict__ st,
                                              AlignState* __restrict__ publish, const TieWords& tw,
                                              const unsigned long long* ticket = nullptr) {
  static_assert(sizeof(AlignState) % 8 == 0, "AlignState is copied in 8-byte words");
  static_assert(offsetof(AlignState, pub) == sizeof(AlignState) - 8, "the publication word is the last 8 bytes");
  static_assert(offsetof(AlignState, iter) % 8 == 0 && offsetof(AlignState, done) == offsetof(AlignState, iter) + 4,
                "iter and done are one 8-byte word");
  __shared__ int tie_s[3];
  if (threadIdx.x == kTieThread) {
    tie_s[0] = tw.pending;
    tie_s[1] = tw.resolved;
    tie_s[2] = tw.err;
  }
  asm volatile("s_waitcnt vmcnt(0)" ::: "memory");
  __syncthreads();
  const auto src = gpw(reinterpret_cast<unsigned long long*>(st));
  const auto dst = gpw(reinterpret_cast<unsigned long long*>(publish));
  constexpr int kWords = (int)(sizeof(AlignState) / 8);
  static_assert(kWords <= 64 * kMomWaves && kLmThreads == 64 * kMomWaves, "one 8-byte word per thread");
  auto patch = [](unsigned long long v, int w, size_t off, int val) {
    if ((size_t)w != off / 8) return v;
    const int sh = (int)(off & 4) * 8;
    return (v & ~(0xffffffffull << sh)) | ((unsigned long long)(unsigned)val << sh);
  };
  __shared__ unsigned long long iter_s;
  const int w = threadIdx.x;
  if (w < kWords) {
    unsigned long long v = __hip_atomic_load(src + w, __ATOMIC_RELAXED, __HIP_MEMORY_SCOPE_AGENT);
    v = patch(v, w, offsetof(AlignState, tie_pending), tie_s[0]);
    v = patch(v, w, offsetof(AlignState, ties_resolved), tie_s[1]);
    v = patch(v, w, offsetof(AlignState, tie_err), tie_s[2]);
    dst[w] = v;
    if (w == (int)(offsetof(AlignState, iter) / 8)) iter_s = v;
  }
  const unsigned long long tk = ticket ? *ticket : job->ticket;
  asm volatile("s_waitcnt vmcnt(0)" ::: "memory");
  __syncthreads();
  if (threadIdx.x == 0) {
    const unsigned long long id = iter_s;
    const unsigned long long w = (tk << 17) | ((unsigned long long)((unsigned)(id >> 32) != 0u) << 16) | (id & 0xffffu);
    __hip_atomic_store(&publish->pub, w, __ATOMIC_RELEASE, __HIP_MEMORY_SCOPE_SYSTEM);
  }
}

template <bool FUSE_LM, bool LOOKUP, bool FRESH>
__device__ __forceinline__ void moments_body(const AlignJob* __restrict__ job, AlignState* __restrict__ st,
                                             AlignState* __restrict__ publish, const FreshStart* fs) {
  static_assert(!FRESH || (FUSE_LM && LOOKUP), "the fresh start exists for the fused one-kernel lookup iteration only");
#ifdef DDLO_MOM_PROF
  unsigned long long mp_t[kMomProfWords] = {0, 0, 0, 0, 0, 0, 0};
#endif
  MOM_PROF(0);
  double R[9], t[3];
  int st_rec, st_any_rec;
  if constexpr (FRESH) {
    for (int e = 0; e < 9; ++e) R[e] = fs->R[e];
    for (int e = 0; e < 3; ++e) t[e] = fs->t[e];
    st_rec = fs->rec0;
    st_any_rec = 0;
    if (blockIdx.x == 0 && threadIdx.x == 64) {
      static_assert(offsetof(AlignJob, guess_t) == offsetof(AlignJob, guess_R) + 72 &&
                        offsetof(AlignJob, job_full) == offsetof(AlignJob, guess_R) + 96 &&
                        offsetof(AlignJob, ticket) == offsetof(AlignJob, guess_R) + 104,
                    "guess_R, guess_t, job_full, ticket: the job's 14 header words");
      AlignJob* const jw = fs->job_w;
      for (int e = 0; e < 9; ++e) jw->guess_R[e] = fs->R[e];
      for (int e = 0; e < 3; ++e) jw->guess_t[e] = fs->t[e];
      jw->job_full = 0;
      jw->ticket = fs->ticket;
    }
  } else {
    const auto sg = gp(st);
    for (int e = 0; e < 9; ++e) R[e] = sg->R[e];
    for (int e = 0; e < 3; ++e) t[e] = sg->t[e];
    st_rec = sg->rec;
    st_any_rec = sg->any_rec;
    if (__builtin_amdgcn_readfirstlane(sg->done)) {
      if (FUSE_LM && publish && blockIdx.x == 0) {
        TieWords tw{};
        if (threadIdx.x == kTieThread) tw = fetch_tie_words(st);
        publish_state(job, st, publish, tw);
      }
      return;
    }
  }
  const CloudDev src = job->src;
  const CloudDev tgt = job->tgt;
  const auto src_cov = gp(job->src_cov);
  const auto tgt_cov = gp(job->tgt_cov);
  const auto key = gp((const unsigned long long*)job->key);
  const auto corr = gpw(job->corr);
  const auto sqd = gpw(job->sqd);
  const auto slab = gpw(job->slab);
  const double max_corr2 = job->max_corr2;
  const int rec = st_rec;
  const int first_rec_done = st_any_rec;
  const int tie_detect = job->tie_detect;
  const bool slice_check = tie_detect && job->tie_scan >= 2 && !(job->tie_ab & 4);
  const bool tie3m = tie_detect && job->tie_scan == 3 && !rec;
  __shared__ NfWaveStack tie_stk[kMomWaves];
  const int lane = lane_id();
  const int wib = threadIdx.x >> 6;
#ifdef DDLO_MOM_PROF
  __builtin_amdgcn_s_waitcnt(0);
#endif
  MOM_PROF(1);
  const int wave = blockIdx.x * kMomWaves + wib;
  const int nwaves_total = gridDim.x * kMomWaves;
  const int ngroups = (src.n + 63) >> 6;
  if (blockIdx.x == 0 && threadIdx.x < kTaskRegions) job->task_ctr[threadIdx.x * kCtrStride] = 0u;
  if (blockIdx.x == 0 && job->grid_on && threadIdx.x == 0) {
    unsigned t = 0;
    for (int sg = 0; sg < kFbSegs; ++sg) t += job->fb_count[sg * 32];
    if constexpr (FRESH) job->fb_count[kFbSegs * 32] = 0u;
    else job->fb_count[kFbSegs * 32] += t;
    for (int sg = 0; sg < kFbSegs; ++sg) job->fb_count[sg * 32] = 0u;
  }
  double acc0 = 0.0, acc1 = 0.0, acc2 = 0.0;
  for (int g = wave; g < ngroups; g += nwaves_total) {
    const int i = g * 64 + lane;
    const bool active = i < src.n;
    int j = -1;
    unsigned kj = 0xffffffffu;
    float kd = INFINITY;
    bool tied = false;
    float4 a = make_float4(0.f, 0.f, 0.f, 0.f), b = a;
    double ca[6] = {0, 0, 0, 0, 0, 0}, cb[6] = {0, 0, 0, 0, 0, 0};
    float lqx = 0.f, lqy = 0.f, lqz = 0.f;
    unsigned long long lkey = 0ull;
    unsigned lsec = 0xffffffffu;
    if constexpr (LOOKUP) {
      const CellGridDev G = job->grid;
      a = ldg4(src.pts, active ? i : src.n - 1);
      const float Rf0 = (float)R[0], Rf1 = (float)R[1], Rf2 = (float)R[2], Rf3 = (float)R[3], Rf4 = (float)R[4],
                  Rf5 = (float)R[5], Rf6 = (float)R[6], Rf7 = (float)R[7], Rf8 = (float)R[8];
      const float tf0 = (float)t[0], tf1 = (float)t[1], tf2 = (float)t[2];
      lqx = (Rf0 * a.x + Rf1 * a.y) + (Rf2 * a.z + tf0);
      lqy = (Rf3 * a.x + Rf4 * a.y) + (Rf5 * a.z + tf1);
      lqz = (Rf6 * a.x + Rf7 * a.y) + (Rf8 * a.z + tf2);
      const int g16 = i >> 4;
      const float qa = job->own_axis == 0 ? lqx : job->own_axis == 1 ? lqy : lqz;
      const bool owned = active && (job->own_axis < 0 || (qa >= job->own_lo && qa < job->own_hi)) &&
                         (job->own_mod == 0 || (g16 % job->own_mod) == job->own_rem);
      unsigned off = 0, cnt = 0;
      if (owned) {
        const float tx = (lqx - G.ox) * G.inv_s, ty = (lqy - G.oy) * G.inv_s, tz = (lqz - G.oz) * G.inv_s;
        if (tx >= 0.f && tx < (float)G.nx && ty >= 0.f && ty < (float)G.ny && tz >= 0.f && tz < (float)G.nz) {
          cg_cell_list(G, tx, ty, tz, off, cnt);
        }
      }
      LookupBest own{~0ull, kLookupInf};
      constexpr int kU = kLookupU;
      auto consume = [&](const float4 (&pp)[kU], unsigned k, unsigned n, float qx, float qy, float qz, LookupBest& r) {
        const unsigned left = n - k;
#pragma unroll
        for (int u = 0; u < kU; ++u) {
          const float dd = dist2(qx, qy, qz, pp[u].x, pp[u].y, pp[u].z);
          const unsigned dw = (unsigned)u < left ? __float_as_uint(dd) : 0xffffffffu;
          const unsigned long long kk = ((unsigned long long)dw << 32) | (unsigned)__float_as_int(pp[u].w);
          const bool take = kk < r.bk;
          r.d2 = min(r.d2, take ? (unsigned)(r.bk >> 32) : dw);
          r.bk = take ? kk : r.bk;
        }
      };
      static_assert(kU <= kCgEntPad, "a round reads at most kCgEntPad entries past a list's end");
      auto fetch = [&](float4 (&pp)[kU], unsigned k, unsigned lo) {
        const float4* const p = G.ent + (size_t)(lo + k);
#pragma unroll
        for (int u = 0; u < kU; ++u) pp[u] = ldg4(p, u);
        __builtin_amdgcn_sched_barrier(0);
      };
      const unsigned c0 = min(cnt, kTailE0);
      for (unsigned k = 0; k < c0; k += kU) {
        float4 pp[kU];
        fetch(pp, k, off);
        consume(pp, k, cnt, lqx, lqy, lqz, own);
      }
      const bool heavy = cnt > kTailE0;
      const unsigned long long rem = __ballot(heavy);
      if (rem != 0ull) {
        const int H = __popcll(rem);
        int lf = 0;
        while ((H << (lf + 1)) <= 64 && (2 << lf) <= kTailFCap) ++lf;
        const int F = 1 << lf;
        const int rank = __popcll(rem & ((1ull << lane) - 1ull));
        int owner = lane;
        if (F > 1) {
          const int team = lane >> lf;
          owner = -1;
          int r = 0;
          for (unsigned long long mm = rem; mm; mm &= mm - 1, ++r)
            if (team == r) owner = __builtin_ctzll(mm);
        }
        const int osrc = owner < 0 ? lane : owner;
        const unsigned ooff = (unsigned)__shfl((int)off, osrc);
        const unsigned ocnt0 = (unsigned)__shfl((int)cnt, osrc);
        const unsigned ocnt = owner < 0 ? 0u : ocnt0;
        const float oqx = __shfl(lqx, osrc), oqy = __shfl(lqy, osrc), oqz = __shfl(lqz, osrc);
        LookupBest mine{~0ull, kLookupInf};
        const unsigned stride = (unsigned)kU << lf;
        unsigned k = kTailE0 + (unsigned)kU * (unsigned)(lane & (F - 1));
#ifdef DDLO_MOM_PROF
        int rounds = 0;
#define MOM_PROF_ROUND ++rounds
#else
#define MOM_PROF_ROUND
#endif
        for (; k < ocnt; k += stride) {
          float4 pp[kU];
          fetch(pp, k, ooff);
          consume(pp, k, ocnt, oqx, oqy, oqz, mine);
          MOM_PROF_ROUND;
        }
#undef MOM_PROF_ROUND
        for (int m = 1; m < F; m <<= 1) tail_merge(mine, tail_shfl(mine, lane ^ m));
        const LookupBest got = tail_shfl(mine, heavy && F > 1 ? rank << lf : lane);
        if (heavy) tail_merge(own, got);
#ifdef DDLO_MOM_PROF
        mp_t[6] = (unsigned long long)H | ((unsigned long long)wave_max((float)rounds) << 8);
#endif
      }
      const unsigned long long bk = own.bk;
      const unsigned d2 = own.d2;
      lkey = owned ? umin64(bk, dkey(job->cap2, -1)) : dkey(INFINITY, -1);
      lsec = (owned && (unsigned)lkey != 0xffffffffu && d2 == (unsigned)(lkey >> 32)) ? (unsigned)(lkey >> 32) : 0xffffffffu;

      MOM_PROF(2);
    }
    if (active) {
      const unsigned long long k = LOOKUP ? lkey : key[i];
      const unsigned sv = !tie_detect ? 0xffffffffu : LOOKUP ? lsec : job->sec[i];
      const unsigned k2lo = (tie3m && !LOOKUP) ? (unsigned)job->key2[i] : 0u;
      kj = (unsigned)k;
      kd = __uint_as_float((unsigned)(k >> 32));
      j = (kj != 0xffffffffu && (double)kd < max_corr2) ? (int)kj : -1;
      if (j >= 0) {
        if constexpr (!LOOKUP) a = ldg4(src.pts, i);
        b = ldg4(tgt.pts, j);
        load_sym6(src_cov + 6 * (size_t)i, ca);
        load_sym6(tgt_cov + 6 * (size_t)j, cb);
      }
      const bool searched = tie_detect && j >= 0 && sv != 0xffffffffu;
      tied = searched && sv <= (unsigned)(k >> 32);
      if (tie3m && searched && !LOOKUP) tied = tied || k2lo != ((unsigned)k ^ 0xffffffffu);
      if (slice_check && searched && !tied) {
        const float qx = ((float)R[0] * a.x + (float)R[1] * a.y) + ((float)R[2] * a.z + (float)t[0]);
        const float qy = ((float)R[3] * a.x + (float)R[4] * a.y) + ((float)R[5] * a.z + (float)t[1]);
        const float qz = ((float)R[6] * a.x + (float)R[7] * a.y) + ((float)R[8] * a.z + (float)t[2]);
        const int b0 = j & ~7;
#pragma unroll
        for (int h = 0; h < 8; ++h) {
          const float4 p = ldg4(tgt.pts, b0 + h);
          tied = tied || (b0 + h != j && dist2(qx, qy, qz, p.x, p.y, p.z) == kd);
        }
      }
    }
    if (tie_detect && __any(tied)) {
      const int j0 = j;
      resolve_tied_corr(job, st, tgt, tied, i, kd, j, &tie_stk[wib], LOOKUP, lqx, lqy, lqz);
      if (tied) kj = (unsigned)j;
      if (j != j0) {
        b = ldg4(tgt.pts, j);
        load_sym6(tgt_cov + 6 * (size_t)j, cb);
      }
    }
    if (active) {
      corr[i] = j;
      sqd[i] = kj != 0xffffffffu ? kd : INFINITY;
      if (rec && !LOOKUP) {
        const float4 qs = ldg4(job->qstate, i);
        if (qs.w >= 0.f) {
          job->ref[i] = make_float4(qs.x, qs.y, qs.z, fminf(__uint_as_float(job->sec[i]), qs.w));
          float4 pp = make_float4(0.f, 0.f, 0.f, __int_as_float(-1));
          if (kj != 0xffffffffu) {
            const float4 p = ldg4(tgt.pts, (int)kj);
            pp = make_float4(p.x, p.y, p.z, __int_as_float((int)kj));
          }
          job->ref_p[i] = pp;
        } else if (!first_rec_done) {
          job->ref[i] = make_float4(0.f, 0.f, 0.f, -1.f);
        }
      }
    }
    Contrib C;
    if (j >= 0) {
      const double A[9] = {ca[0], ca[1], ca[2], ca[1], ca[3], ca[4], ca[2], ca[4], ca[5]};
      double RC[9];
#pragma unroll
      for (int r = 0; r < 3; ++r)
#pragma unroll
        for (int cc = 0; cc < 3; ++cc) RC[3 * r + cc] = R[3 * r] * A[cc] + R[3 * r + 1] * A[3 + cc] + R[3 * r + 2] * A[6 + cc];
      double S[9];
#pragma unroll
      for (int r = 0; r < 3; ++r)
#pragma unroll
        for (int cc = 0; cc < 3; ++cc) S[3 * r + cc] = RC[3 * r] * R[3 * cc] + RC[3 * r + 1] * R[3 * cc + 1] + RC[3 * r + 2] * R[3 * cc + 2];
      const double Cm[9] = {cb[0] + S[0], cb[1] + S[1], cb[2] + S[2], cb[1] + S[3], cb[3] + S[4],
                            cb[4] + S[5], cb[2] + S[6], cb[4] + S[7], cb[5] + S[8]};
      double Mi[9];
      inv3(Cm, Mi);
      C.M[0] = Mi[0]; C.M[1] = 0.5 * (Mi[1] + Mi[3]); C.M[2] = 0.5 * (Mi[2] + Mi[6]);
      C.M[3] = Mi[4]; C.M[4] = 0.5 * (Mi[5] + Mi[7]); C.M[5] = Mi[8];
      const double ax = a.x, ay = a.y, az = a.z;
      C.q[0] = (R[0] * ax + R[1] * ay) + (R[2] * az + t[0]);
      C.q[1] = (R[3] * ax + R[4] * ay) + (R[5] * az + t[1]);
      C.q[2] = (R[6] * ax + R[7] * ay) + (R[8] * az + t[2]);
      const double e0 = (double)b.x - C.q[0], e1 = (double)b.y - C.q[1], e2 = (double)b.z - C.q[2];
      C.v[0] = C.M[0] * e0 + C.M[1] * e1 + C.M[2] * e2;
      C.v[1] = C.M[1] * e0 + C.M[3] * e1 + C.M[4] * e2;
      C.v[2] = C.M[2] * e0 + C.M[4] * e1 + C.M[5] * e2;
      C.y = e0 * C.v[0] + e1 * C.v[1] + e2 * C.v[2];
      C.c = 1.0;
    } else {
      for (int e = 0; e < 6; ++e) C.M[e] = 0.0;
      C.q[0] = C.q[1] = C.q[2] = 0.0;
      C.v[0] = C.v[1] = C.v[2] = 0.0;
      C.y = 0.0;
      C.c = 0.0;
    }
    C.qq[0] = C.q[0] * C.q[0]; C.qq[1] = C.q[0] * C.q[1]; C.qq[2] = C.q[0] * C.q[2];
    C.qq[3] = C.q[1] * C.q[1]; C.qq[4] = C.q[1] * C.q[2]; C.qq[5] = C.q[2] * C.q[2];
    MOM_PROF(3);
    acc0 += final_pair(treduce<5, 0>(C));
    acc1 += final_pair(treduce<5, 1>(C));
    acc2 += final_pair(treduce<5, 2>(C));
  }
  MOM_PROF(4);
  __shared__ double red[kMomWaves][kMomentSlots];
  if ((lane & 1) == 0) {
    const int base = moment_base(lane);
    red[wib][base + 0] = acc0;
    red[wib][base + 1] = acc1;
    red[wib][base + 2] = acc2;
  }
  __syncthreads();
  if (threadIdx.x < kSlabStride) {
    double sum = 0.0;
    if (threadIdx.x < kMoments)
      for (int w = 0; w < kMomWaves; ++w) sum += red[w][threadIdx.x];
    if constexpr (FUSE_LM)
      __hip_atomic_store((__attribute__((address_space(1))) unsigned long long*)(slab + (size_t)blockIdx.x * kSlabStride +
                                                                                 threadIdx.x),
                         (unsigned long long)__double_as_longlong(sum), __ATOMIC_RELAXED, __HIP_MEMORY_SCOPE_AGENT);
    else
      slab[(size_t)blockIdx.x * kSlabStride + threadIdx.x] = sum;
  }
#ifdef DDLO_MOM_PROF
  MOM_PROF(5);
  if (LOOKUP && lane == 0 && wave < kMomProfWaves) {
    unsigned long long* o = g_mom_prof + ((size_t)min(st->iter, kMomProfIters - 1) * kMomProfWaves + wave) * kMomProfWords;
    for (int e = 0; e < kMomProfWords; ++e) o[e] = mp_t[e];
  }
#endif
  if constexpr (FUSE_LM) {
    __shared__ int last_s;
    asm volatile("s_waitcnt vmcnt(0)" ::: "memory");
    __syncthreads();
    unsigned* const arrive = job->task_ctr + kTaskRegions * kCtrStride;
    if (threadIdx.x == 0) last_s = atomicAdd(arrive, 1u) == gridDim.x - 1;
    __syncthreads();
    if (!last_s) return;
    if (threadIdx.x == 0) {
      __builtin_amdgcn_fence(__ATOMIC_ACQUIRE, "agent");
      asm volatile("s_waitcnt vmcnt(0)" ::: "memory");
      atomicExch(arrive, 0u);
    }
    __syncthreads();
    TieWords tw{};
    if (publish && threadIdx.x == kTieThread) tw = fetch_tie_words(st);
    lm_step_body<false, FRESH>(job, st, job->slab, job->nblocks, nullptr, fs);
    if (publish) publish_state(job, st, publish, tw, FRESH ? &fs->ticket : nullptr);
  }
}

template <bool FUSE_LM, bool LOOKUP = false>
__global__ __launch_bounds__(64 * kMomWaves) void k_moments(const AlignJob* __restrict__ job,
                                                            AlignState* __restrict__ st, AlignState* __restrict__ publish) {
  moments_body<FUSE_LM, LOOKUP, false>(job, st, publish, nullptr);
}
__global__ __launch_bounds__(64 * kMomWaves) void k_moments_fresh(const AlignJob* __restrict__ job,
                                                                  AlignState* __restrict__ st,
                                                                  AlignState* __restrict__ publish, const FreshStart fs) {
  moments_body<true, true, true>(job, st, publish, &fs);
}
template __global__ void k_moments<false>(const AlignJob*, AlignState*, AlignState*);
template __global__ void k_moments<true>(const AlignJob*, AlignState*, AlignState*);
template __global__ void k_moments<false, true>(const AlignJob*, AlignState*, AlignState*);
template __global__ void k_moments<true, true>(const AlignJob*, AlignState*, AlignState*);

__global__ __launch_bounds__(kLmThreads) void k_mom_reduce(const AlignJob* __restrict__ job) {
  AlignState* st = job->state;
  if (__builtin_amdgcn_readfirstlane(st->done)) return;
  __shared__ double part[kLmParts][kSlabStride];
  __shared__ double mom[kSlabStride];
  reduce_slab(job->slab, job->nblocks, part, mom);
  __syncthreads();
  if (threadIdx.x < kSlabStride) gpw(job->mom)[threadIdx.x] = mom[threadIdx.x];
}

__global__ __launch_bounds__(kLmThreads) void k_lm_step(const AlignJob* __restrict__ job, AlignState* __restrict__ st,
                                                        const double* __restrict__ slab, int nblocks,
                                                        const double* __restrict__ premom,
                                                        AlignState* __restrict__ publish) {
  TieWords tw{};
  if (publish && threadIdx.x == kTieThread) tw = fetch_tie_words(st);
  if (!__builtin_amdgcn_readfirstlane(st->done)) {
    if (premom) lm_step_body<true>(job, st, slab, nblocks, premom);
    else lm_step_body<false>(job, st, slab, nblocks, nullptr);
  }
  if (publish) publish_state(job, st, publish, tw);
}

bool linearize_is_one_kernel(const LinGeom& g) {
  static const int fused_lookup = env_knob("DDLO_GRID_FUSED", 1);
  return g.grid && !g.grid_walk && fused_lookup;
}
void launch_linearize(hipStream_t s, const AlignJob* job, const LinGeom& g, AlignState* publish) {
  if (linearize_is_one_kernel(g)) {
    if (g.fuse_lm) k_moments<true, true><<<g.mom_blocks, 64 * kMomWaves, 0, s>>>(job, g.state, publish);
    else k_moments<false, true><<<g.mom_blocks, 64 * kMomWaves, 0, s>>>(job, g.state, nullptr);
    return;
  }
  if (g.grid) launch_cell_lookup(s, job, g);
  if (!g.grid || g.grid_walk) launch_nn_walk(s, job, g);
  if (g.fuse_lm) k_moments<true><<<g.mom_blocks, 64 * kMomWaves, 0, s>>>(job, g.state, publish);
  else k_moments<false><<<g.mom_blocks, 64 * kMomWaves, 0, s>>>(job, g.state, nullptr);
}
void launch_linearize_fresh(hipStream_t s, const AlignJob* job, const LinGeom& g, const FreshStart& fs,
                            AlignState* publish) {
  k_moments_fresh<<<g.mom_blocks, 64 * kMomWaves, 0, s>>>(job, g.state, publish, fs);
}
int moment_blocks(int nsrc) {
  const int groups = (nsrc + 63) / 64;
  return std::max(1, std::min((groups + kMomWaves - 1) / kMomWaves, kMomBlocksMax));
}
int lm_slab_rows_max() { return kMomBlocksMax; }
void launch_lm_step(hipStream_t s, const AlignJob* job, AlignState* st, const double* slab, int nblocks,
                    const double* premom, AlignState* publish) {
  k_lm_step<<<1, kLmThreads, 0, s>>>(job, st, slab, nblocks, premom, publish);
}
void launch_mom_reduce(hipStream_t s, const AlignJob* job) { k_mom_reduce<<<1, kLmThreads, 0, s>>>(job); }

}

#ifdef DDLO_MOM_PROF
extern "C" int ddlo_dev_mom_prof(unsigned long long* out) {
  return (int)hipMemcpyFromSymbol(out, HIP_SYMBOL(ddlo::g_mom_prof), sizeof(ddlo::g_mom_prof));
}
#endif
```

Baseline: 37130 GICP iters/s.

## Pass fused GICP job parameters as kernel arguments instead of device job loads

Gathers the parameters the fused moments/LM kernel needs into a 256-byte FusedArgs block. On the fresh-start path and its follow-on iterations, the block is passed by value as a kernel argument so it arrives in scalar registers, instead of being loaded from the device AlignJob struct. Inline asm pins these fields, and the R/t state loads, in SGPR/VGPR to avoid reloads and serialized scalar loads at kernel start. The aim is to shorten the start-up latency of each iteration kernel. The cost is higher scalar register pressure and a larger kernel-argument payload per launch.

```diff
diff --git a/dynamic_direct_lidar_odometry_amd/csrc/align.hip b/dynamic_direct_lidar_odometry_amd/csrc/align.hip
--- a/dynamic_direct_lidar_odometry_amd/csrc/align.hip
+++ b/dynamic_direct_lidar_odometry_amd/csrc/align.hip
@@ -78,6 +78,7 @@
 
 void ddlo::rt::finalize_job(gicp_ctx* c) {
   AlignJob& j = *c->job_host;
+  fill_fused_args(j);
   j.job_full = 0;
   AlignJob probe = j;
   std::memcpy(probe.guess_R, c->job_last.guess_R, sizeof(probe.guess_R));
@@ -183,6 +184,46 @@
   return GICP_OK;
 }
 
+void ddlo::rt::fill_fused_args(AlignJob& j) {
+  FusedArgs& f = j.fused;
+  std::memset(&f, 0, sizeof(f));
+  f.src_pts = j.src.pts;
+  f.tgt_pts = j.tgt.pts;
+  f.tgt_inv_perm = j.tgt.inv_perm;
+  f.src_cov = j.src_cov;
+  f.tgt_cov = j.tgt_cov;
+  f.corr = j.corr;
+  f.sqd = j.sqd;
+  f.slab = j.slab;
+  f.task_ctr = j.task_ctr;
+  f.fb_count = j.fb_count;
+  f.grid = j.grid;
+  f.max_corr2 = j.max_corr2;
+  f.lm_init_lambda_factor = j.lm_init_lambda_factor;
+  f.transformation_epsilon = j.transformation_epsilon;
+  f.rotation_epsilon = j.rotation_epsilon;
+  f.src_n = j.src.n;
+  f.tgt_n = j.tgt.n;
+  f.nblocks = j.nblocks;
+  f.cap2 = j.cap2;
+  f.own_axis = j.own_axis;
+  f.own_lo = j.own_lo;
+  f.own_hi = j.own_hi;
+  f.own_mod = j.own_mod;
+  f.own_rem = j.own_rem;
+  f.tie_detect = j.tie_detect;
+  f.tie_scan = j.tie_scan;
+  f.tie_ab = j.tie_ab;
+  f.grid_on = j.grid_on;
+  f.optimizer = j.optimizer;
+  f.max_iterations = j.max_iterations;
+  f.fixed_iterations = j.fixed_iterations;
+  f.lm_max_iterations = j.lm_max_iterations;
+  f.reuse = j.reuse;
+  f.reuse_rec_eps = j.reuse_rec_eps;
+  f.reuse_rec_conv = j.reuse_rec_conv;
+}
+
 namespace {
 
 LinGeom geometry(const gicp_ctx* c) {
@@ -252,10 +293,13 @@
   return GICP_OK;
 }
 
-gicp_status ddlo::rt::enqueue_iteration(gicp_ctx* c, const AlignJob* jd, int nblocks, AlignState* publish) {
+gicp_status ddlo::rt::enqueue_iteration(gicp_ctx* c, const AlignJob* jd, int nblocks, AlignState* publish, bool args) {
   (void)nblocks;
   const LinGeom g = geometry(c);
-  launch_linearize(c->stream, jd, g, publish);
+  if (args && linearize_is_one_kernel(g) && g.fuse_lm)
+    launch_linearize_args(c->stream, jd, g, c->job_host->fused, c->job_host->ticket, publish);
+  else
+    launch_linearize(c->stream, jd, g, publish);
   if (c->comm) {
     launch_mom_reduce(c->stream, jd);
     NCCL_TRY(rccl().all_reduce(c->mom.p, c->mom.p, kSlabStride, ncclFloat64, ncclSum, c->comm, c->stream));
@@ -268,11 +312,11 @@
 
 namespace {
 
-gicp_status enqueue_chunk(gicp_ctx* c, bool with_init, int iters, int nblocks, int slot) {
+gicp_status enqueue_chunk(gicp_ctx* c, bool with_init, int iters, int nblocks, int slot, bool args = false) {
   AlignJob* jd = c->job_dev.as<AlignJob>();
   if (with_init) launch_align_init(c->stream, jd, c->job_host_dev);
   for (int i = 0; i < iters; ++i) {
-    gicp_status s = enqueue_iteration(c, jd, nblocks, i == iters - 1 ? c->state_host_dev + slot : nullptr);
+    gicp_status s = enqueue_iteration(c, jd, nblocks, i == iters - 1 ? c->state_host_dev + slot : nullptr, args);
     if (s) return s;
   }
   return GICP_OK;
@@ -369,9 +413,9 @@
       fs.ticket = jh.ticket;
       fs.job_w = c->job_dev.as<AlignJob>();
       fs.rec0 = jh.reuse && jh.reuse_rec0;
-      launch_linearize_fresh(c->stream, c->job_dev.as<AlignJob>(), g, fs, first == 1 ? c->state_host_dev : nullptr);
+      launch_linearize_fresh(c->stream, c->job_dev.as<AlignJob>(), g, fs, jh.fused, first == 1 ? c->state_host_dev : nullptr);
       HIP_TRY(hipGetLastError());
-      return first > 1 ? enqueue_chunk(c, false, first - 1, nblocks, 0) : GICP_OK;
+      return first > 1 ? enqueue_chunk(c, false, first - 1, nblocks, 0, true) : GICP_OK;
     }
     if (use_graph) {
       HIP_TRY(hipGraphLaunch(is_first ? gs->first[first - 1].ge : gs->rest[k & 1].ge, c->stream));
diff --git a/dynamic_direct_lidar_odometry_amd/csrc/capi_debug.hip b/dynamic_direct_lidar_odometry_amd/csrc/capi_debug.hip
--- a/dynamic_direct_lidar_odometry_amd/csrc/capi_debug.hip
+++ b/dynamic_direct_lidar_odometry_amd/csrc/capi_debug.hip
@@ -58,6 +58,7 @@
   j.fixed_iterations = c->dbg_job.fixed_iterations;
   j.job_full = c->dbg_job.job_full;
   j.ticket = c->dbg_job.ticket;
+  fill_fused_args(j);
   const bool same = std::memcmp(&j, &c->dbg_job, sizeof(AlignJob)) == 0;
   std::memcpy(&j, &c->dbg_job, sizeof(AlignJob));
   if (!same) {
@@ -303,6 +304,7 @@
   j.transformation_epsilon = c->params.transformation_epsilon;
   j.rotation_epsilon = c->params.rotation_epsilon;
   j.reuse = 0;
+  fill_fused_args(j);
   AlignState st{};
   std::memcpy(st.R, in->R, sizeof(st.R));
   std::memcpy(st.t, in->t, sizeof(st.t));
diff --git a/dynamic_direct_lidar_odometry_amd/csrc/capi_internal.hpp b/dynamic_direct_lidar_odometry_amd/csrc/capi_internal.hpp
--- a/dynamic_direct_lidar_odometry_amd/csrc/capi_internal.hpp
+++ b/dynamic_direct_lidar_odometry_amd/csrc/capi_internal.hpp
@@ -50,9 +50,10 @@
 };
 void finalize_job(gicp_ctx* c);
 gicp_status fill_job(gicp_ctx* c, const float* guess16, int nblocks);
+void fill_fused_args(AlignJob& j);
 gicp_status prepare_align(gicp_ctx* c);
 gicp_status ensure_tie_tree(gicp_ctx* c);
-gicp_status enqueue_iteration(gicp_ctx* c, const AlignJob* jd, int nblocks, AlignState* publish);
+gicp_status enqueue_iteration(gicp_ctx* c, const AlignJob* jd, int nblocks, AlignState* publish, bool args = false);
 void drop_graphs(gicp_ctx* c);
 
 
diff --git a/dynamic_direct_lidar_odometry_amd/csrc/gicp_types.hpp b/dynamic_direct_lidar_odometry_amd/csrc/gicp_types.hpp
--- a/dynamic_direct_lidar_odometry_amd/csrc/gicp_types.hpp
+++ b/dynamic_direct_lidar_odometry_amd/csrc/gicp_types.hpp
@@ -98,6 +98,33 @@
   cnt = (unsigned)(e >> 32) & 0x3fffffffu;
   return 1;
 }
+
+struct FusedArgs {
+  const float4* src_pts;
+  const float4* tgt_pts;
+  const int* tgt_inv_perm;
+  const double* src_cov;
+  const double* tgt_cov;
+  int* corr;
+  float* sqd;
+  double* slab;
+  unsigned* task_ctr;
+  unsigned* fb_count;
+  CellGridDev grid;
+  double max_corr2;
+  double lm_init_lambda_factor, transformation_epsilon, rotation_epsilon;
+  int src_n, tgt_n;
+  int nblocks;
+  float cap2;
+  int own_axis;
+  float own_lo, own_hi;
+  int own_mod, own_rem;
+  int tie_detect, tie_scan, tie_ab, grid_on;
+  int optimizer, max_iterations, fixed_iterations, lm_max_iterations;
+  int reuse;
+  float reuse_rec_eps, reuse_rec_conv;
+};
+static_assert(sizeof(FusedArgs) == 256, "FusedArgs: 64 dwords, no hidden padding");
 
 struct AlignState {
   double R[9];
@@ -189,6 +216,7 @@
   int* fb_list;
   int fb_seg_cap;
   unsigned short* fb_mask;
+  FusedArgs fused;
 };
 constexpr int kFbSegs = 8;
 
diff --git a/dynamic_direct_lidar_odometry_amd/csrc/launch.hpp b/dynamic_direct_lidar_odometry_amd/csrc/launch.hpp
--- a/dynamic_direct_lidar_odometry_amd/csrc/launch.hpp
+++ b/dynamic_direct_lidar_odometry_amd/csrc/launch.hpp
@@ -47,7 +47,9 @@
 void launch_linearize(hipStream_t s, const AlignJob* job, const LinGeom& g, AlignState* publish = nullptr);
 bool linearize_is_one_kernel(const LinGeom& g);
 void launch_linearize_fresh(hipStream_t s, const AlignJob* job, const LinGeom& g, const FreshStart& fs,
-                            AlignState* publish = nullptr);
+                            const FusedArgs& fa, AlignState* publish = nullptr);
+void launch_linearize_args(hipStream_t s, const AlignJob* job, const LinGeom& g, const FusedArgs& fa,
+                           unsigned long long ticket, AlignState* publish = nullptr);
 int search_queries_per_wave();
 int task_cap_per_region(int nsrc);
 int moment_blocks(int nsrc);
diff --git a/dynamic_direct_lidar_odometry_amd/csrc/lm_step.hpp b/dynamic_direct_lidar_odometry_amd/csrc/lm_step.hpp
--- a/dynamic_direct_lidar_odometry_amd/csrc/lm_step.hpp
+++ b/dynamic_direct_lidar_odometry_amd/csrc/lm_step.hpp
@@ -241,7 +241,7 @@
 #define LM_PROF_TRIAL(i)
 #endif
 template <bool PREMOM, bool FRESH = false>
-__device__ __forceinline__ void lm_step_body(const AlignJob* __restrict__ job, AlignState* __restrict__ st,
+__device__ __forceinline__ void lm_step_body(const FusedArgs& fa, AlignState* __restrict__ st,
                                              const double* __restrict__ slab, int nblocks,
                                              const double* __restrict__ premom, const FreshStart* fs = nullptr) {
 #ifdef DDLO_LM_PROF
@@ -274,12 +274,12 @@
   } else {
     if (tid < 12) rt_v = tid < 9 ? st->R[tid] : st->t[tid - 9];
   }
-  const int optimizer = job->optimizer, lm_max_iterations = job->lm_max_iterations;
-  const int fixed_iterations = job->fixed_iterations, max_iterations = job->max_iterations;
-  const double lm_init_lambda_factor = job->lm_init_lambda_factor;
-  const double rotation_epsilon = job->rotation_epsilon, transformation_epsilon = job->transformation_epsilon;
-  const int reuse = job->reuse;
-  const float reuse_rec_eps = job->reuse_rec_eps, reuse_rec_conv = job->reuse_rec_conv;
+  const int optimizer = fa.optimizer, lm_max_iterations = fa.lm_max_iterations;
+  const int fixed_iterations = fa.fixed_iterations, max_iterations = fa.max_iterations;
+  const double lm_init_lambda_factor = fa.lm_init_lambda_factor;
+  const double rotation_epsilon = fa.rotation_epsilon, transformation_epsilon = fa.transformation_epsilon;
+  const int reuse = fa.reuse;
+  const float reuse_rec_eps = fa.reuse_rec_eps, reuse_rec_conv = fa.reuse_rec_conv;
   NeqTerm E{};
   if (tid < kNeqEntries) E = kNeq.e[tid];
   if constexpr (PREMOM) {
diff --git a/dynamic_direct_lidar_odometry_amd/csrc/moments.hip b/dynamic_direct_lidar_odometry_amd/csrc/moments.hip
--- a/dynamic_direct_lidar_odometry_amd/csrc/moments.hip
+++ b/dynamic_direct_lidar_odometry_amd/csrc/moments.hip
@@ -123,8 +123,8 @@
 
 constexpr int kMomWaves = 8;
 
-__device__ __forceinline__ void resolve_tied_corr(const AlignJob* __restrict__ job, AlignState* st, const CloudDev& tgt,
-                                               bool tied, int i, float kd, int& j, NfWaveStack* S,
+__device__ __forceinline__ void resolve_tied_corr(const AlignJob* __restrict__ job, AlignState* st,
+                                               const int* tgt_inv_perm, bool tied, int i, float kd, int& j, NfWaveStack* S,
                                                bool q_in_regs = false, float qx = 0.f, float qy = 0.f, float qz = 0.f) {
   unsigned long long tm = __ballot(tied);
   const int lane = lane_id();
@@ -153,7 +153,7 @@
     rix = __builtin_amdgcn_readfirstlane(rix);
     if (!ok) err = 1;
     else if (__float_as_uint(rd) != __float_as_uint(dl) || rix < 0 || rix >= t.n) err = 16;
-    else if ((jn = tgt.inv_perm[rix]) < 0) err = 32;
+    else if ((jn = tgt_inv_perm[rix]) < 0) err = 32;
     if (lane == l) {
       if (jn >= 0) j = jn;
       else atomicOr(&st->tie_err, err);
@@ -264,10 +264,36 @@
   }
 }
 
-template <bool FUSE_LM, bool LOOKUP, bool FRESH>
+__device__ __forceinline__ void hold_fused_args(FusedArgs& f) {
+  asm volatile("" :: "s"(f.src_pts), "s"(f.tgt_pts), "s"(f.src_cov), "s"(f.tgt_cov), "s"(f.corr), "s"(f.sqd),
+               "s"(f.grid.dir), "s"(f.grid.fine), "s"(f.grid.ent), "s"(f.grid.ox), "s"(f.grid.oy), "s"(f.grid.oz),
+               "s"(f.grid.inv_s), "s"(f.grid.nx), "s"(f.grid.ny), "s"(f.grid.nz), "s"(f.max_corr2), "s"(f.src_n),
+               "s"(f.cap2), "s"(f.own_axis), "s"(f.own_lo), "s"(f.own_hi), "s"(f.own_mod), "s"(f.own_rem),
+               "s"(f.tie_detect), "s"(f.tie_scan), "s"(f.tie_ab));
+  asm volatile("" : "+s"(f.src_pts), "+s"(f.tgt_pts), "+s"(f.src_cov), "+s"(f.tgt_cov), "+s"(f.corr), "+s"(f.sqd),
+               "+s"(f.grid.dir), "+s"(f.grid.fine), "+s"(f.grid.ent), "+s"(f.grid.ox), "+s"(f.grid.oy),
+               "+s"(f.grid.oz), "+s"(f.grid.inv_s), "+s"(f.grid.nx), "+s"(f.grid.ny));
+  asm volatile("" : "+s"(f.grid.nz), "+s"(f.max_corr2), "+s"(f.src_n), "+s"(f.cap2), "+s"(f.own_axis), "+s"(f.own_lo),
+               "+s"(f.own_hi), "+s"(f.own_mod), "+s"(f.own_rem), "+s"(f.tie_detect), "+s"(f.tie_scan), "+s"(f.tie_ab));
+}
+__device__ __forceinline__ void hold_fused_tail(FusedArgs& f) {
+  asm volatile("" : "+s"(f.slab), "+s"(f.task_ctr), "+s"(f.nblocks), "+s"(f.lm_init_lambda_factor),
+               "+s"(f.transformation_epsilon), "+s"(f.rotation_epsilon), "+s"(f.optimizer), "+s"(f.max_iterations),
+               "+s"(f.fixed_iterations), "+s"(f.lm_max_iterations), "+s"(f.reuse), "+s"(f.reuse_rec_eps),
+               "+s"(f.reuse_rec_conv));
+}
+
+template <bool FUSE_LM, bool LOOKUP, bool FRESH, bool ARGS = false>
 __device__ __forceinline__ void moments_body(const AlignJob* __restrict__ job, AlignState* __restrict__ st,
-                                             AlignState* __restrict__ publish, const FreshStart* fs) {
+                                             AlignState* __restrict__ publish, const FreshStart* fs,
+                                             const FusedArgs* ka = nullptr, const unsigned long long* ticket = nullptr) {
   static_assert(!FRESH || (FUSE_LM && LOOKUP), "the fresh start exists for the fused one-kernel lookup iteration only");
+  static_assert(!ARGS || (FUSE_LM && LOOKUP), "the argument block exists for the fused one-kernel lookup iteration only");
+  static_assert(!FRESH || ARGS, "a fresh start is a plain launch");
+  constexpr bool kBatch = FUSE_LM && LOOKUP;
+  FusedArgs fb;
+  if constexpr (kBatch) fb = ARGS ? *ka : job->fused;
+  const FusedArgs& fa = kBatch ? fb : job->fused;
 #ifdef DDLO_MOM_PROF
   unsigned long long mp_t[kMomProfWords] = {0, 0, 0, 0, 0, 0, 0};
 #endif
@@ -279,6 +305,9 @@
     for (int e = 0; e < 3; ++e) t[e] = fs->t[e];
     st_rec = fs->rec0;
     st_any_rec = 0;
+    asm volatile("" : "+v"(R[0]), "+v"(R[1]), "+v"(R[2]), "+v"(R[3]), "+v"(R[4]), "+v"(R[5]), "+v"(R[6]), "+v"(R[7]),
+                 "+v"(R[8]), "+v"(t[0]), "+v"(t[1]), "+v"(t[2]));
+    hold_fused_args(fb);
     if (blockIdx.x == 0 && threadIdx.x == 64) {
       static_assert(offsetof(AlignJob, guess_t) == offsetof(AlignJob, guess_R) + 72 &&
                         offsetof(AlignJob, job_full) == offsetof(AlignJob, guess_R) + 96 &&
@@ -292,33 +321,52 @@
     }
   } else {
     const auto sg = gp(st);
-    for (int e = 0; e < 9; ++e) R[e] = sg->R[e];
-    for (int e = 0; e < 3; ++e) t[e] = sg->t[e];
+    if constexpr (kBatch) {
+      int vz = 0;
+      asm volatile("" : "+v"(vz));
+      static_assert(offsetof(AlignState, t) == offsetof(AlignState, R) + 72, "R, t: 12 consecutive doubles");
+      const auto Rt = gp(&st->R[0]);
+      for (int e = 0; e < 9; ++e) R[e] = Rt[e + vz];
+      for (int e = 0; e < 3; ++e) t[e] = Rt[9 + e + vz];
+    } else {
+      for (int e = 0; e < 9; ++e) R[e] = sg->R[e];
+      for (int e = 0; e < 3; ++e) t[e] = sg->t[e];
+    }
     st_rec = sg->rec;
     st_any_rec = sg->any_rec;
-    if (__builtin_amdgcn_readfirstlane(sg->done)) {
+    const int st_done = sg->done;
+    if constexpr (kBatch) {
+      asm volatile("" : "+v"(R[0]), "+v"(R[1]), "+v"(R[2]), "+v"(R[3]), "+v"(R[4]), "+v"(R[5]), "+v"(R[6]), "+v"(R[7]),
+                   "+v"(R[8]), "+v"(t[0]), "+v"(t[1]), "+v"(t[2]) : "s"(st_rec), "s"(st_any_rec), "s"(st_done));
+      hold_fused_args(fb);
+    }
+    if (__builtin_amdgcn_readfirstlane(st_done)) {
       if (FUSE_LM && publish && blockIdx.x == 0) {
         TieWords tw{};
         if (threadIdx.x == kTieThread) tw = fetch_tie_words(st);
-        publish_state(job, st, publish, tw);
+        publish_state(job, st, publish, tw, ticket);
       }
       return;
     }
   }
-  const CloudDev src = job->src;
-  const CloudDev tgt = job->tgt;
-  const auto src_cov = gp(job->src_cov);
-  const auto tgt_cov = gp(job->tgt_cov);
-  const auto key = gp((const unsigned long long*)job->key);
-  const auto corr = gpw(job->corr);
-  const auto sqd = gpw(job->sqd);
-  const auto slab = gpw(job->slab);
-  const double max_corr2 = job->max_corr2;
+  struct {
+    const float4* pts;
+    int n;
+  } const src{fa.src_pts, fa.src_n}, tgt{fa.tgt_pts, fa.tgt_n};
+  const auto src_cov = gp(fa.src_cov);
+  const auto tgt_cov = gp(fa.tgt_cov);
+  const unsigned long long* key_p = nullptr;
+  if constexpr (!LOOKUP) key_p = job->key;
+  const auto key = gp(key_p);
+  const auto corr = gpw(fa.corr);
+  const auto sqd = gpw(fa.sqd);
+  const auto slab = gpw(fa.slab);
+  const double max_corr2 = fa.max_corr2;
   const int rec = st_rec;
   const int first_rec_done = st_any_rec;
-  const int tie_detect = job->tie_detect;
-  const bool slice_check = tie_detect && job->tie_scan >= 2 && !(job->tie_ab & 4);
-  const bool tie3m = tie_detect && job->tie_scan == 3 && !rec;
+  const int tie_detect = fa.tie_detect;
+  const bool slice_check = tie_detect && fa.tie_scan >= 2 && !(fa.tie_ab & 4);
+  const bool tie3m = tie_detect && fa.tie_scan == 3 && !rec;
   __shared__ NfWaveStack tie_stk[kMomWaves];
   const int lane = lane_id();
   const int wib = threadIdx.x >> 6;
@@ -329,13 +377,13 @@
   const int wave = blockIdx.x * kMomWaves + wib;
   const int nwaves_total = gridDim.x * kMomWaves;
   const int ngroups = (src.n + 63) >> 6;
-  if (blockIdx.x == 0 && threadIdx.x < kTaskRegions) job->task_ctr[threadIdx.x * kCtrStride] = 0u;
-  if (blockIdx.x == 0 && job->grid_on && threadIdx.x == 0) {
+  if (blockIdx.x == 0 && threadIdx.x < kTaskRegions) fa.task_ctr[threadIdx.x * kCtrStride] = 0u;
+  if (blockIdx.x == 0 && fa.grid_on && threadIdx.x == 0) {
     unsigned t = 0;
-    for (int sg = 0; sg < kFbSegs; ++sg) t += job->fb_count[sg * 32];
-    if constexpr (FRESH) job->fb_count[kFbSegs * 32] = 0u;
-    else job->fb_count[kFbSegs * 32] += t;
-    for (int sg = 0; sg < kFbSegs; ++sg) job->fb_count[sg * 32] = 0u;
+    for (int sg = 0; sg < kFbSegs; ++sg) t += fa.fb_count[sg * 32];
+    if constexpr (FRESH) fa.fb_count[kFbSegs * 32] = 0u;
+    else fa.fb_count[kFbSegs * 32] += t;
+    for (int sg = 0; sg < kFbSegs; ++sg) fa.fb_count[sg * 32] = 0u;
   }
   double acc0 = 0.0, acc1 = 0.0, acc2 = 0.0;
   for (int g = wave; g < ngroups; g += nwaves_total) {
@@ -351,7 +399,7 @@
     unsigned long long lkey = 0ull;
     unsigned lsec = 0xffffffffu;
     if constexpr (LOOKUP) {
-      const CellGridDev G = job->grid;
+      const CellGridDev G = fa.grid;
       a = ldg4(src.pts, active ? i : src.n - 1);
       const float Rf0 = (float)R[0], Rf1 = (float)R[1], Rf2 = (float)R[2], Rf3 = (float)R[3], Rf4 = (float)R[4],
                   Rf5 = (float)R[5], Rf6 = (float)R[6], Rf7 = (float)R[7], Rf8 = (float)R[8];
@@ -360,9 +408,9 @@
       lqy = (Rf3 * a.x + Rf4 * a.y) + (Rf5 * a.z + tf1);
       lqz = (Rf6 * a.x + Rf7 * a.y) + (Rf8 * a.z + tf2);
       const int g16 = i >> 4;
-      const float qa = job->own_axis == 0 ? lqx : job->own_axis == 1 ? lqy : lqz;
-      const bool owned = active && (job->own_axis < 0 || (qa >= job->own_lo && qa < job->own_hi)) &&
-                         (job->own_mod == 0 || (g16 % job->own_mod) == job->own_rem);
+      const float qa = fa.own_axis == 0 ? lqx : fa.own_axis == 1 ? lqy : lqz;
+      const bool owned = active && (fa.own_axis < 0 || (qa >= fa.own_lo && qa < fa.own_hi)) &&
+                         (fa.own_mod == 0 || (g16 % fa.own_mod) == fa.own_rem);
       unsigned off = 0, cnt = 0;
       if (owned) {
         const float tx = (lqx - G.ox) * G.inv_s, ty = (lqy - G.oy) * G.inv_s, tz = (lqz - G.oz) * G.inv_s;
@@ -443,7 +491,7 @@
       }
       const unsigned long long bk = own.bk;
       const unsigned d2 = own.d2;
-      lkey = owned ? umin64(bk, dkey(job->cap2, -1)) : dkey(INFINITY, -1);
+      lkey = owned ? umin64(bk, dkey(fa.cap2, -1)) : dkey(INFINITY, -1);
       lsec = (owned && (unsigned)lkey != 0xffffffffu && d2 == (unsigned)(lkey >> 32)) ? (unsigned)(lkey >> 32) : 0xffffffffu;
 
       MOM_PROF(2);
@@ -478,7 +526,7 @@
     }
     if (tie_detect && __any(tied)) {
       const int j0 = j;
-      resolve_tied_corr(job, st, tgt, tied, i, kd, j, &tie_stk[wib], LOOKUP, lqx, lqy, lqz);
+      resolve_tied_corr(job, st, fa.tgt_inv_perm, tied, i, kd, j, &tie_stk[wib], LOOKUP, lqx, lqy, lqz);
       if (tied) kj = (unsigned)j;
       if (j != j0) {
         b = ldg4(tgt.pts, j);
@@ -547,6 +595,7 @@
     acc2 += final_pair(treduce<5, 2>(C));
   }
   MOM_PROF(4);
+  if constexpr (kBatch) hold_fused_tail(fb);
   __shared__ double red[kMomWaves][kMomentSlots];
   if ((lane & 1) == 0) {
     const int base = moment_base(lane);
@@ -577,7 +626,7 @@
     __shared__ int last_s;
     asm volatile("s_waitcnt vmcnt(0)" ::: "memory");
     __syncthreads();
-    unsigned* const arrive = job->task_ctr + kTaskRegions * kCtrStride;
+    unsigned* const arrive = fa.task_ctr + kTaskRegions * kCtrStride;
     if (threadIdx.x == 0) last_s = atomicAdd(arrive, 1u) == gridDim.x - 1;
     __syncthreads();
     if (!last_s) return;
@@ -589,8 +638,8 @@
     __syncthreads();
     TieWords tw{};
     if (publish && threadIdx.x == kTieThread) tw = fetch_tie_words(st);
-    lm_step_body<false, FRESH>(job, st, job->slab, job->nblocks, nullptr, fs);
-    if (publish) publish_state(job, st, publish, tw, FRESH ? &fs->ticket : nullptr);
+    lm_step_body<false, FRESH>(fa, st, fa.slab, fa.nblocks, nullptr, fs);
+    if (publish) publish_state(job, st, publish, tw, FRESH ? &fs->ticket : ticket);
   }
 }
 
@@ -601,8 +650,15 @@
 }
 __global__ __launch_bounds__(64 * kMomWaves) void k_moments_fresh(const AlignJob* __restrict__ job,
                                                                   AlignState* __restrict__ st,
-                                                                  AlignState* __restrict__ publish, const FreshStart fs) {
-  moments_body<true, true, true>(job, st, publish, &fs);
+                                                                  AlignState* __restrict__ publish, const FreshStart fs,
+                                                                  const FusedArgs fa) {
+  moments_body<true, true, true, true>(job, st, publish, &fs, &fa);
+}
+__global__ __launch_bounds__(64 * kMomWaves) void k_moments_args(const AlignJob* __restrict__ job,
+                                                                 AlignState* __restrict__ st,
+                                                                 AlignState* __restrict__ publish, const FusedArgs fa,
+                                                                 const unsigned long long ticket) {
+  moments_body<true, true, false, true>(job, st, publish, nullptr, &fa, &ticket);
 }
 template __global__ void k_moments<false>(const AlignJob*, AlignState*, AlignState*);
 template __global__ void k_moments<true>(const AlignJob*, AlignState*, AlignState*);
@@ -626,8 +682,8 @@
   TieWords tw{};
   if (publish && threadIdx.x == kTieThread) tw = fetch_tie_words(st);
   if (!__builtin_amdgcn_readfirstlane(st->done)) {
-    if (premom) lm_step_body<true>(job, st, slab, nblocks, premom);
-    else lm_step_body<false>(job, st, slab, nblocks, nullptr);
+    if (premom) lm_step_body<true>(job->fused, st, slab, nblocks, premom);
+    else lm_step_body<false>(job->fused, st, slab, nblocks, nullptr);
   }
   if (publish) publish_state(job, st, publish, tw);
 }
@@ -648,8 +704,12 @@
   else k_moments<false><<<g.mom_blocks, 64 * kMomWaves, 0, s>>>(job, g.state, nullptr);
 }
 void launch_linearize_fresh(hipStream_t s, const AlignJob* job, const LinGeom& g, const FreshStart& fs,
-                            AlignState* publish) {
-  k_moments_fresh<<<g.mom_blocks, 64 * kMomWaves, 0, s>>>(job, g.state, publish, fs);
+                            const FusedArgs& fa, AlignState* publish) {
+  k_moments_fresh<<<g.mom_blocks, 64 * kMomWaves, 0, s>>>(job, g.state, publish, fs, fa);
+}
+void launch_linearize_args(hipStream_t s, const AlignJob* job, const LinGeom& g, const FusedArgs& fa,
+                           unsigned long long ticket, AlignState* publish) {
+  k_moments_args<<<g.mom_blocks, 64 * kMomWaves, 0, s>>>(job, g.state, publish, fa, ticket);
 }
 int moment_blocks(int nsrc) {
   const int groups = (nsrc + 63) / 64;
```

New measurement: 38100 GICP iters/s (median of 6 runs). +2.6%, better.
